# cristianpjensen/thesis-pai-reconstruction

Hardware: AMD Instinct MI355X
Metric: train images/sec (256x256, bs=64) Pix2Pix step (higher is better)
Workload: dtype bf16; 1 GPU; Pix2Pix generator+PatchGAN GAN step, 256x256x1 pairs, 64 images/GPU (BASELINE configs[1]); global_batch=64, per_gpu_batch=64, loss_type=gan, parallelism=dp1, grad_bucket_dtype=f32

## Files before the change

### include/pai_hip.h

```cpp
#ifndef PAI_HIP_H
#define PAI_HIP_H

#include <stdint.h>

#ifdef __cplusplus
extern "C" {
#endif

#define PAI_F32 0
#define PAI_BF16 1
#define PAI_U8 2

#define PAI_ACT_NONE 0
#define PAI_ACT_LRELU 1
#define PAI_ACT_RELU 2
#define PAI_ACT_TANH 3
#define PAI_ACT_SILU 4

const char* pai_last_error(void);
int pai_version(void);
int pai_build_flags(void);
int pai_device_info(int* cu_count, int* lds_bytes, char* arch_name, int arch_name_len);

#define PAI_TUNABLE_UNSET (-2147483647 - 1)
int pai_set_tunable(const char* name, int value);

typedef struct pai_conv_desc {
    int32_t dtype;
    int32_t transposed;
    int32_t N, H, W;
    int32_t C1, C2;
    int32_t Cout;
    int32_t kernel;
    int32_t stride;
    int32_t pad;
    int32_t relu1, relu2;
    int32_t epilogue_act;
    int32_t groups;
    int32_t pack_flags;
    int32_t hints;
} pai_conv_desc;
#define PAI_HINT_SOLO 1

int pai_conv_out_hw(const pai_conv_desc* d, int* OH, int* OW);
int pai_conv_fwd_stats_rows(const pai_conv_desc* d);
int pai_conv_fwd_stats_rows_max(const pai_conv_desc* d);
int pai_bn_stats_buffer_rows(int rows);

int pai_conv_kernel_id(const pai_conv_desc* d, int op);
int pai_conv_kernel_name(const pai_conv_desc* d, int op, char* name, int name_len);

int pai_create(int device_id, void** handle_out);
int pai_bind(void* handle);
int pai_destroy(void* handle);
int pai_handle_set_workspace(void* handle, void* zeroed_device_memory, int64_t bytes);
int pai_handle_set_scratch(void* handle, void* device_memory, int64_t bytes);
int pai_handle_set_wgrad_workspace(void* handle, void* device_memory, int64_t bytes);

int pai_set_workspace(void* zeroed_device_memory, int64_t bytes);
int64_t pai_conv_workspace_bytes(const pai_conv_desc* d, int op);
int pai_set_scratch(void* device_memory, int64_t bytes);
int64_t pai_conv_scratch_bytes(const pai_conv_desc* d, int op);
int pai_set_wgrad_workspace(void* device_memory, int64_t bytes);
int64_t pai_conv_wgrad_workspace_bytes(const pai_conv_desc* d);

int pai_conv_fwd(const pai_conv_desc* d, const void* x1, const void* x2, const void* w_fwd,
                 const float* bias, void* y_raw, void* y_act, float* y_f32, float* stats,
                 void* stream);

int pai_conv_dgrad(const pai_conv_desc* d, const void* dy, const void* w_dgrad, void* dx1,
                   void* dx2, int only_c2, void* stream);

int pai_conv_dgrad_f32add_ok(const pai_conv_desc* d);
int pai_conv_dgrad_f32add(const pai_conv_desc* d, const void* dy, const void* w_dgrad, const float* addend,
                          float* dx2_f32, void* stream);

int pai_conv_dgrad_act(const pai_conv_desc* d, const void* dy, const void* w_dgrad, void* dx1,
                       void* dx2, const void* a1, int act1, void* stream);

typedef struct pai_bwd_epilogue {
    const void* z;
    const void* add;
    const float* scale;
    const float* shift;
    const float* mean;
    const float* rstd;
    float* partials;
    int32_t act1, act2;
} pai_bwd_epilogue;
int pai_conv_dgrad_bn_rows_max(const pai_conv_desc* d);
int pai_conv_dgrad_bn(const pai_conv_desc* d, const void* dy, const void* w_dgrad, void* dx1,
                      void* dx2, const pai_bwd_epilogue* e, int* partial_rows, void* stream);

typedef struct pai_bn_train {
    const float* gamma;
    const float* beta;
    float eps, momentum;
    int32_t n_updates;
    float* running_mean;
    float* running_var;
    int64_t* num_batches_tracked;
    float *mean, *rstd, *scale, *shift;
} pai_bn_train;
int pai_conv_fwd_bn(const pai_conv_desc* d, const void* x1, const void* x2, const void* w_fwd, const float* bias,
                    void* z, void* a, int act, const pai_bn_train* bn, float* stats, void* stream);
int pai_conv_dgrad_bn_apply(const pai_conv_desc* d, const void* dy, const void* w_dgrad, void* du_scratch, void* dx2,
                            const pai_bwd_epilogue* e, const float* gamma, float* sums, float* dgamma, float* dbeta,
                            void* dz, void* stream);
int pai_conv_bn_fused(const pai_conv_desc* d, int op);

int pai_conv_wgrad(const pai_conv_desc* d, const void* x1, const void* x2, const void* dy,
                   float* dw, float* dbias, void* stream);
int pai_conv_wgrad_overwrite(const pai_conv_desc* d, const void* x1, const void* x2, const void* dy,
                             float* dw, float* dbias, void* stream);
int pai_conv_wgrad_overwrite_w(const pai_conv_desc* d, const void* x1, const void* x2, const void* dy,
                               float* dw, float* dbias, void* stream);

int pai_conv_prologue_ok(const pai_conv_desc* d);
int pai_conv_fwd_pro(const pai_conv_desc* d, const void* x1, const void* w_fwd, const float* bias, void* y_raw,
                     float* stats, const float* pre_scale, const float* pre_shift, int pre_act, void* stream);
int pai_conv_wgrad_pro(const pai_conv_desc* d, const void* x1, const void* dy, float* dw, float* dbias, int overwrite,
                       const float* pre_scale, const float* pre_shift, int pre_act, void* stream);

int pai_pack_weights(int dtype, const float* w_master, int Cout, int taps, int Cin,
                     void* w_fwd_or_null, void* w_dgrad_or_null, void* stream);
int pai_pack_weights_multi(int n, const float* const* w_master, const int32_t* cout, const int32_t* taps,
                           const int32_t* cin, void* const* w_fwd, void* const* w_dgrad, void* stream);

int pai_bn_finalize(const float* stats, int rows, int C, int64_t count, const float* gamma,
                    const float* beta, float eps, float momentum, int n_updates,
                    float* running_mean, float* running_var, int64_t* num_batches_tracked,
                    float* mean, float* rstd, float* scale, float* shift, void* stream);
int pai_bn_eval_coeffs(int C, const float* gamma, const float* beta, const float* running_mean,
                       const float* running_var, float eps, float* scale, float* shift,
                       void* stream);
int pai_bn_apply(int dtype, const void* z, int64_t M, int C, const float* scale,
                 const float* shift, int act, void* out, void* stream);
int pai_bn2_add_act(int dtype, const void* za, const float* scale_a, const float* shift_a, const void* zb,
                    const float* scale_b, const float* shift_b, int64_t M, int C, int act_a, int act, void* out,
                    void* stream);
int pai_bn_bwd_partial_rows(int64_t M);
int pai_bn_bwd_reduce(int dtype, const void* g1, int act1, const void* g2, int act2, const void* a,
                      const void* z, int64_t M, int C, const float* mean, const float* rstd,
                      void* du, float* partials, float* sums, float* dgamma, float* dbeta,
                      void* stream);
int pai_bn_bwd_reduce_affine(int dtype, const void* g1, int act1, const void* g2, int act2, const void* z,
                             int64_t M, int C, const float* scale, const float* shift, const float* mean,
                             const float* rstd, void* du, float* partials, float* sums, float* dgamma,
                             float* dbeta, void* stream);
int pai_bn_bwd_finalize(const float* partials, int rows, int C, float* sums, float* dgamma,
                        float* dbeta, void* stream);
int pai_bn_bwd_apply(int dtype, const void* du, const void* z, int64_t M, int C,
                     const float* mean, const float* rstd, const float* gamma,
                     const float* sums, void* dz, void* stream);
int pai_bn_bwd_apply_affine(int dtype, const void* g1, int act1, const void* z, int64_t M, int C, const float* scale,
                            const float* shift, const float* mean, const float* rstd, const float* gamma,
                            const float* sums, void* dz, void* stream);
int pai_act_bwd(int dtype, const void* g1, int act1, const void* g2, int act2, const void* a,
                int64_t numel, void* du, void* stream);

int pai_dropout2d(int dtype, const void* x, const float* mask, int N, int64_t HW, int C, void* out,
                  void* stream);

int pai_maxpool2(int dtype, const void* x, int N, int H, int W, int C, void* out, unsigned char* idx, void* stream);
int pai_maxpool2_bwd(int dtype, const void* dout, const unsigned char* idx, int N, int H, int W, int C, void* dx,
                     void* stream);
int pai_upsample2(int dtype, const void* x, int N, int H, int W, int C, void* out, void* stream);
int pai_upsample2_bwd(int dtype, const void* dout, int N, int H, int W, int C, void* dx, void* stream);
int pai_add_act(int dtype, const void* a, const void* b, int64_t numel, int act, void* out, void* stream);
int pai_bn2_bwd_reduce(int dtype, const void* d, int act_a, const void* za, const void* zb, int64_t M, int C,
                       const float* scale_a, const float* shift_a, const float* mean_a, const float* rstd_a,
                       const float* mean_b, const float* rstd_b, float* part_a, float* part_b, float* sums_a, float* sums_b,
                       void* stream);
int pai_bn2_bwd_apply(int dtype, const void* d, int act_a, const void* za, const void* zb, int64_t M, int C,
                      const float* scale_a, const float* shift_a, const float* mean_a, const float* rstd_a,
                      const float* gamma_a, const float* sums_a, const float* mean_b, const float* rstd_b,
                      const float* gamma_b, const float* sums_b, void* dza, void* dzb, void* stream);
int pai_instnorm_fwd(int dtype, const void* x, int N, int HW, int C, float eps, int act, void* y, float* mean, float* rstd,
                     void* stream);
int pai_instnorm_bwd(int dtype, const void* g, const void* x, int N, int HW, int C, int act, const float* mean,
                     const float* rstd, void* dx, void* stream);

int pai_layernorm_partial_rows(int64_t M);
int pai_layernorm_fwd(int dtype, const void* x, const void* res, int64_t M, int D, const float* gamma,
                      const float* beta, float eps, const float* post, int P, void* sum_out, void* y,
                      float* mean, float* rstd, void* stream);
int pai_layernorm_bwd(int dtype, const void* dy, const void* xs, int64_t M, int D, const float* gamma,
                      const float* mean, const float* rstd, void* dx, float* dgamma_dbeta, float* partials,
                      void* stream);
int pai_gelu(int dtype, const void* z, int64_t numel, void* out, void* stream);
int pai_gelu_bwd(int dtype, const void* dy, const void* z, int64_t numel, void* dz, void* stream);
int pai_mha_fwd(int dtype, const void* qkv, int S, int B, int heads, int hd, const float* mask, void* out,
                float* probs, void* stream);
int pai_mha_bwd(int dtype, const void* dout, const void* qkv, const float* probs, int S, int B, int heads,
                int hd, const float* mask, void* dqkv, float* ds_workspace, void* stream);
int pai_mha_kernel_name(int dtype, int S, int hd, int op, char* name, int name_len);
int pai_subsample2(int dtype, const void* x, int N, int H, int W, int C, void* out, void* stream);
int pai_subsample2_bwd(int dtype, const void* dout, int N, int H, int W, int C, void* dx, void* stream);
int pai_bn_stats_rows(int64_t M);
int pai_bn_stats(int dtype, const void* z, int64_t M, int C, float* stats, void* stream);
int pai_colsum(int dtype, const void* x, int64_t rows, int C, float* out, void* stream);

int pai_gate_partial_rows(int64_t M);
int pai_gate_hidden(int dtype, const void* ig, const void* sg, int64_t M, int K, const float* scale_i,
                    const float* shift_i, const float* scale_s, const float* shift_s, const float* w_a,
                    const float* b_a, void* h, float* logit, float* partials, void* stream);
int pai_gate_apply(int dtype, const void* x, const float* logit, int64_t M, int C, const float* scale_a,
                   const float* shift_a, void* out, float* att, void* stream);
int pai_gate_apply_bwd(int dtype, const void* dout, const void* x, const float* att, const float* logit,
                       int64_t M, int C, const float* mean_a, const float* rstd_a, void* dx_skip, float* dl,
                       float* partials, int relu_out, void* stream);
int pai_gate_hidden_bwd(int dtype, const float* dl, const float* logit, const void* h, const void* ig,
                        const void* sg, int64_t M, int K, const float* mean_a, const float* rstd_a,
                        const float* gamma_a, const float* sums_a, const float* w_a, const float* mean_i,
                        const float* rstd_i, const float* mean_s, const float* rstd_s, void* dsum,
                        float* partials_i, float* partials_s, float* dw_a, float* db_a, void* stream);

int pai_bce_logits(const float* logits, int64_t numel, float target, float loss_scale,
                   double* loss, float grad_scale, float* grad, void* stream);
int pai_l1(const float* pred, const float* target, int64_t numel, float loss_scale, double* loss,
           float grad_scale, float* grad, void* stream);
int pai_mse(const float* pred, const float* target, int64_t numel, float loss_scale, double* loss,
            float grad_scale, float* grad, void* stream);
int pai_head_loss_ok(const pai_conv_desc* d, int has_bias);
int pai_head_loss(const pai_conv_desc* d, const void* a3, const void* w_fwd, const void* w_dgrad, int n_first,
                  float target_first, float target_rest, float loss_scale, double* loss, float grad_scale,
                  float* logits, void* dl, float* dl_f32, void* du, const void* act_src, int act, void* stream);
int pai_scalar_take(double* acc, float* out, void* stream);
int pai_metrics_take(double* sums, int64_t n_images, int64_t numel, float* out3, void* stream);
int pai_tanh_bwd(int dtype, const float* pred, const float* g_a, const float* g_b, int64_t numel,
                 void* dh, void* stream);

int pai_denormalize(const float* x, const float* grad_out_or_null, int64_t numel, float* out,
                    void* stream);

int pai_ssim_sse(const float* pred, const float* target, int NC, int H, int W, int denorm,
                 double* out2, double* per_image, float* full_map, void* stream);
int pai_ssim_psnr_bwd(const float* pred, const float* target, int NC, int H, int W, int denorm,
                      float w_ssim, float w_psnr, const double* sse, float* grad, float* workspace,
                      void* stream);
int64_t pai_ssim_bwd_workspace_floats(int NC, int H, int W);
int pai_eval_planes(const float* pred, const float* target, int NC, int H, int W, int denorm,
                    double* ssim_plane, double* sse_plane, unsigned char* ssim_map_u8,
                    const unsigned char* lut_rgb, unsigned char* hot_u8, void* stream);
int pai_eval_kernel_name(int op, char* name, int name_len);

int pai_cast(int src_dtype, const void* src, int dst_dtype, void* dst, int64_t numel, void* stream);
int pai_reduce_rows(const float* partial, int rows, int C, float* out, int accumulate, void* stream);
int pai_adam(float* param, const float* grad, float* exp_avg, float* exp_avg_sq, int64_t numel,
             float lr, float beta1, float beta2, float eps, int step_count, void* stream);
int pai_adam_pack(float* param, const float* grad, float* exp_avg, float* exp_avg_sq, int64_t numel, int64_t w_off,
                  int Cout, int taps, int Cin, void* w_fwd, void* w_dgrad, float lr, float beta1, float beta2, float eps,
                  int step_count, void* stream);
int pai_adam_dev(float* param, const float* grad, float* exp_avg, float* exp_avg_sq, int64_t numel,
                 float lr, float beta1, float beta2, float eps, int64_t* step_dev, float* coeff2_dev, void* stream);
int pai_adam_multi(int count, void* const* params, const void* const* grads, void* const* exp_avgs,
                   void* const* exp_avg_sqs, const int64_t* numels, float lr, float beta1, float beta2, float eps,
                   int step_count, void* stream);
int pai_adam_multi_dev(int count, void* const* params, const void* const* grads, void* const* exp_avgs,
                       void* const* exp_avg_sqs, const int64_t* numels, float lr, float beta1, float beta2, float eps,
                       int64_t* step_dev, float* coeff2_dev, void* stream);

#define PAI_COMM_ID_BYTES 128
int pai_comm_unique_id(void* id_out_host);
int pai_comm_init(const void* id_host, int rank, int world, void** comm_out);
int pai_allreduce(void* comm, void* ptr, int64_t count, int dtype, void* stream);
int pai_comm_destroy(void* comm);

typedef struct pai_plan_s* pai_plan_t;
int pai_plan_create(pai_plan_t* out);
int pai_plan_destroy(pai_plan_t plan);
int pai_plan_begin(pai_plan_t plan);
int pai_plan_end(pai_plan_t plan);
int pai_plan_run(pai_plan_t plan, int64_t step_delta);
int pai_plan_info(pai_plan_t plan, int* launches, int* waits, int* streams, int64_t* runs);
int pai_stream_wait(void* waiting_stream, void* signalling_stream);
int pai_stream_wait_last(void* waiting_stream, void* signalling_stream);
typedef struct pai_event_s* pai_event_t;
int pai_event_create(pai_event_t* out);
int pai_event_destroy(pai_event_t ev);
int pai_event_record(pai_event_t ev, void* stream);
int pai_event_create_timing(pai_event_t* out);
int pai_event_elapsed_ms(pai_event_t start, pai_event_t stop, float* ms_host);
int pai_profile_arm(pai_event_t start, pai_event_t stop);
int pai_stream_wait_event(void* waiting_stream, pai_event_t ev);
int pai_zero_multi(int count, void* const* ptrs, const int64_t* numels, void* stream);
int pai_cast_multi(int count, int src_dtype, const void* const* srcs, int dst_dtype, void* const* dsts,
                   const int64_t* numels, void* stream);
int pai_lerp_multi(int count, void* const* dsts, const void* const* srcs, const int64_t* numels, float weight, void* stream);

int pai_filter_to_dense(const float* w_oihw, int Cout, int Cin_per_group, int taps, int groups, float* dense, void* stream);
int pai_filter_grad_from_dense(const float* dense_dw, int Cout, int Cin_per_group, int taps, int groups, float* dw_oihw,
                               void* stream);

int pai_swap_mid(int elem_bytes, const void* src, int64_t A, int B, int C, int64_t D, void* dst, void* stream);
int pai_scale(float* ptr, int64_t numel, float factor, void* stream);

int pai_resize_aa_u8(const void* src, int n, int H, int W, int S, const int* wbounds, const float* wweights, int KW,
                     const int* hbounds, const float* hweights, int KH, const int* hbounds_host, void* dst, void* stream);
int pai_batch_gather(int src_dtype, const void* cache_a, const void* cache_b, int64_t M, int64_t per_image,
                     const int64_t* indices, int count, const float* table, float* out_a, float* out_b, void* stream);
int pai_data_kernel_name(int op, int src_dtype, char* name, int name_len);

int pai_sattn_fwd(int dtype, const void* qkv, int N, int T, int heads, int ch, void* out, void* stream);
int pai_sattn_fwd_lse(int dtype, const void* qkv, int N, int T, int heads, int ch, void* out, float* lse, void* stream);
int pai_sattn_bwd(int dtype, const void* dout, const void* qkv, const void* out, const float* lse, int N, int T, int heads,
                  int ch, void* dqkv, float* ws, void* stream);
int pai_sattn_kernel_name(int dtype, int ch, int op, char* name, int name_len);
int pai_affine_act(int dtype, const void* x, int64_t rows_per_sample, int N, int C, const float* A, const float* B,
                   int per_sample, int act, void* out, void* stream);
// ... 22 lines not shown
```

### thesis-pai-reconstruction_amd/csrc/api.hip

```cpp
#include <stdarg.h>

#include "common.h"

static thread_local char g_err[512] = "";

void pai_set_error(const char* fmt, ...) {
    va_list ap;
    va_start(ap, fmt);
    vsnprintf(g_err, sizeof(g_err), fmt, ap);
    va_end(ap);
}

extern "C" const char* pai_last_error(void) { return g_err; }
extern "C" int pai_version(void) { return 140; }

extern "C" int pai_build_flags(void) { return 0; }

extern "C" int pai_device_info(int* cu_count, int* lds_bytes, char* arch_name, int arch_name_len) {
    int dev = 0;
    hipError_t e = hipGetDevice(&dev);
    PAI_CHECK(e == hipSuccess, "hipGetDevice: %s", hipGetErrorString(e));
    hipDeviceProp_t p;
    e = hipGetDeviceProperties(&p, dev);
    PAI_CHECK(e == hipSuccess, "hipGetDeviceProperties: %s", hipGetErrorString(e));
    if (cu_count) *cu_count = p.multiProcessorCount;
    if (lds_bytes) *lds_bytes = (int)p.sharedMemPerBlock;
    if (arch_name && arch_name_len > 0) {
        strncpy(arch_name, p.gcnArchName, arch_name_len - 1);
        arch_name[arch_name_len - 1] = 0;
    }
    return 0;
}

struct Tunable { char name[32]; int value; };
static Tunable g_tunables[32];
static int g_ntunables = 0;

struct TunableEnv { char name[32]; int has, value; };
static TunableEnv g_tunable_env[48];
static int g_ntunable_env = 0;
static bool tunable_env(const char* name, int* value) {
    for (int i = 0; i < g_ntunable_env; ++i)
        if (!strcmp(g_tunable_env[i].name, name)) { *value = g_tunable_env[i].value; return g_tunable_env[i].has != 0; }
    char key[64];
    snprintf(key, sizeof(key), "PAI_TUNE_%s", name);
    const char* e = getenv(key);
    if (g_ntunable_env < 48 && strlen(name) < sizeof(g_tunable_env[0].name)) {
        TunableEnv& t = g_tunable_env[g_ntunable_env];
        strcpy(t.name, name);
        t.has = e != nullptr;
        t.value = e ? atoi(e) : 0;
        ++g_ntunable_env;
    }
    *value = e ? atoi(e) : 0;
    return e != nullptr;
}

int pai_tunable(const char* name, int def) {
    for (int i = 0; i < g_ntunables; ++i)
        if (!strcmp(g_tunables[i].name, name)) return g_tunables[i].value;
    int v;
    return tunable_env(name, &v) ? v : def;
}

extern "C" int pai_set_tunable(const char* name, int value) {
    PAI_CHECK(name && strlen(name) < sizeof(g_tunables[0].name), "pai_set_tunable: bad name");
    for (int i = 0; i < g_ntunables; ++i)
        if (!strcmp(g_tunables[i].name, name)) {
            if (value == PAI_TUNABLE_UNSET) g_tunables[i] = g_tunables[--g_ntunables];
            else g_tunables[i].value = value;
            return 0;
        }
    if (value == PAI_TUNABLE_UNSET) return 0;
    PAI_CHECK(g_ntunables < 32, "pai_set_tunable: table full");
    strcpy(g_tunables[g_ntunables].name, name);
    g_tunables[g_ntunables++].value = value;
    return 0;
}

static void finish_gg(GG* g);

static int check_desc(const pai_conv_desc* d) {
    PAI_CHECK(d != nullptr, "null descriptor");
    PAI_CHECK(d->dtype == PAI_F32 || d->dtype == PAI_BF16, "bad dtype %d", d->dtype);
    if (d->kernel == 1) {
        PAI_CHECK(d->pad == 0 && d->stride == 1 && !d->transposed, "kernel=1 needs pad=0 stride=1 Conv2d");
    } else if (d->kernel == 3) {
        PAI_CHECK(d->pad == 1 && d->stride == 1 && !d->transposed, "kernel=3 needs pad=1 stride=1 Conv2d");
    } else {
        PAI_CHECK(d->kernel == 4 && d->pad == 1, "only kernel=4 pad=1 or kernel=1 pad=0 supported (got k=%d p=%d)",
                  d->kernel, d->pad);
    }
    PAI_CHECK(d->N > 0 && d->H > 0 && d->W > 0 && d->C1 > 0 && d->C2 >= 0 && d->Cout > 0,
              "bad shape N=%d H=%d W=%d C1=%d C2=%d Cout=%d", d->N, d->H, d->W, d->C1, d->C2,
              d->Cout);
    if (d->transposed) {
        PAI_CHECK(d->stride == 2, "ConvTranspose2d needs stride 2");
// ... 467 lines not shown

extern "C" int pai_conv_fwd_pro(const pai_conv_desc* d, const void* x1, const void* w_fwd, const float* bias, void* y_raw,
                                float* stats, const float* pre_scale, const float* pre_shift, int pre_act, void* stream) {
    GG g;
    if (gg_build_fwd(d, &g)) return 1;
    PAI_CHECK(x1 && w_fwd && y_raw && pre_scale && pre_shift, "pai_conv_fwd_pro: null pointer");
    PAI_CHECK(pre_act == PAI_ACT_NONE || pre_act == PAI_ACT_RELU, "pai_conv_fwd_pro: pre_act=%d (none or ReLU)", pre_act);
    PAI_CHECK(d->C2 == 0, "pai_conv_fwd_pro: one source tensor only");
    FwdArgs a;
    memset(&a, 0, sizeof(a));
    a.x1 = x1; a.w = w_fwd; a.bias = bias;
    a.y1 = y_raw;
    a.stats = stats;
    a.pscale = pre_scale; a.pshift = pre_shift; a.pact = pre_act;
    return run_fwd(d->dtype, g, a, (hipStream_t)stream);
}

extern "C" int pai_conv_wgrad_pro(const pai_conv_desc* d, const void* x1, const void* dy, float* dw, float* dbias,
                                  int overwrite, const float* pre_scale, const float* pre_shift, int pre_act, void* stream) {
    PAI_CHECK(pre_scale && pre_shift, "pai_conv_wgrad_pro: null prologue");
    PAI_CHECK(pre_act == PAI_ACT_NONE || pre_act == PAI_ACT_RELU, "pai_conv_wgrad_pro: pre_act=%d (none or ReLU)", pre_act);
    PAI_CHECK(d->C2 == 0, "pai_conv_wgrad_pro: one source tensor only");
    return conv_wgrad_impl(d, x1, nullptr, dy, dw, dbias, overwrite ? 1 : 0, stream, pre_scale, pre_shift, pre_act);
}

extern "C" int pai_conv_dgrad(const pai_conv_desc* d, const void* dy, const void* w_dgrad,
                              void* dx1, void* dx2, int only_c2, void* stream) {
    GG g;
    if (gg_build_dgrad(d, &g)) return 1;
    PAI_CHECK(dy && w_dgrad, "pai_conv_dgrad: null dy / w");
    PAI_CHECK(only_c2 ? (dx2 && d->C2 > 0) : (dx1 != nullptr), "pai_conv_dgrad: missing output");
    PAI_CHECK(d->C2 == 0 || dx2, "pai_conv_dgrad: C2 > 0 but dx2 is null");
    FwdArgs a;
    memset(&a, 0, sizeof(a));
    a.x1 = dy; a.w = w_dgrad;
    a.y1 = dx1; a.y2 = dx2;
    a.skip_d1 = only_c2;
    return run_fwd(d->dtype, g, a, (hipStream_t)stream);
}

extern "C" int pai_conv_dgrad_f32add_ok(const pai_conv_desc* d) {
    GG g;
    if (!d || gg_build_dgrad(d, &g)) return 0;
    return pai_tunable("head_fused", 1) && thin_up_f32add_ok(d->dtype, g) ? 1 : 0;
}

extern "C" int pai_conv_dgrad_f32add(const pai_conv_desc* d, const void* dy, const void* w_dgrad, const float* addend,
                                     float* dx2_f32, void* stream) {
    GG g;
    if (gg_build_dgrad(d, &g)) return 1;
    PAI_CHECK(dy && w_dgrad && addend && dx2_f32, "pai_conv_dgrad_f32add: null pointer");
    PAI_CHECK(thin_up_f32add_ok(d->dtype, g), "pai_conv_dgrad_f32add: not a bf16 (1 | 1)-channel k4 s2 layer on thin_up_k (ask pai_conv_dgrad_f32add_ok)");
    FwdArgs a;
    memset(&a, 0, sizeof(a));
    a.x1 = dy; a.w = w_dgrad;
    a.yf32 = dx2_f32; a.badd = addend;
    a.skip_d1 = 1;
    return launch_thin_dgrad(g, a, (hipStream_t)stream);
}

extern "C" int pai_conv_dgrad_act(const pai_conv_desc* d, const void* dy, const void* w_dgrad,
                                  void* dx1, void* dx2, const void* a1, int act1, void* stream) {
    GG g;
    if (gg_build_dgrad(d, &g)) return 1;
    PAI_CHECK(dy && w_dgrad && dx1 && a1, "pai_conv_dgrad_act: null pointer");
    PAI_CHECK(d->C2 == 0 || dx2, "pai_conv_dgrad_act: C2 > 0 but dx2 is null");
    PAI_CHECK(act1 == PAI_ACT_LRELU || act1 == PAI_ACT_RELU || act1 == PAI_ACT_NONE, "pai_conv_dgrad_act: act1=%d", act1);
    FwdArgs a;
    memset(&a, 0, sizeof(a));
    a.x1 = dy; a.w = w_dgrad;
    a.y1 = dx1; a.y2 = dx2;
    hipStream_t s = (hipStream_t)stream;
    FwdPick p = pick_fwd(d->dtype, g, a);
    const bool fused = p.fused || p.k == FK_HEAD_DGRAD;
    if (fused) {
        a.bz = a1; a.bact1 = act1;
        p = pick_fwd(d->dtype, g, a);
    }
    int rc = run_fwd(p, d->dtype, g, a, s);
    if (rc || fused || act1 == PAI_ACT_NONE) return rc;
    return pai_act_bwd(d->dtype, dx1, act1, nullptr, PAI_ACT_NONE, a1, (int64_t)g.N * g.OH * g.OW * g.D1, dx1, stream);
}

extern "C" int pai_conv_dgrad_bn_rows_max(const pai_conv_desc* d) {
    GG g;
    if (gg_build_dgrad(d, &g)) return -1;
    int fused = cdiv(g.M, 16) * g.nphase;
    if (pw_rows(g) > fused) fused = pw_rows(g);
    if (pwx_rows(g) > fused) fused = pwx_rows(g);
    const int twopass = pai_bn_bwd_partial_rows((int64_t)g.N * g.OH * g.OW);
    return fused > twopass ? fused : twopass;
}

int bn_bwd_reduce_affine(int dtype, void* g1_du, int act1, const void* g2, int act2, const void* z, int64_t M, int C,
                         const float* scale, const float* shift, const float* mean, const float* rstd,
                         float* partials, hipStream_t s);

extern "C" int pai_conv_dgrad_bn(const pai_conv_desc* d, const void* dy, const void* w_dgrad, void* dx1,
                                 void* dx2, const pai_bwd_epilogue* e, int* partial_rows, void* stream) {
    GG g;
    if (gg_build_dgrad(d, &g)) return 1;
    PAI_CHECK(dy && w_dgrad && dx1 && e && e->z, "pai_conv_dgrad_bn: null pointer");
    PAI_CHECK(d->C2 == 0 || dx2, "pai_conv_dgrad_bn: C2 > 0 but dx2 is null");
    PAI_CHECK((e->scale == nullptr) == (e->shift == nullptr), "pai_conv_dgrad_bn: scale and shift go together");
    PAI_CHECK(!e->partials || (e->mean && e->rstd && partial_rows), "pai_conv_dgrad_bn: partials need mean, rstd and partial_rows");
    for (int act : {e->act1, e->act2})
        PAI_CHECK(act == PAI_ACT_LRELU || act == PAI_ACT_RELU || act == PAI_ACT_NONE, "pai_conv_dgrad_bn: act=%d", act);
    FwdArgs a;
    memset(&a, 0, sizeof(a));
    a.x1 = dy; a.w = w_dgrad;
    a.y1 = dx1; a.y2 = dx2;
    hipStream_t s = (hipStream_t)stream;
    const int64_t M = (int64_t)g.N * g.OH * g.OW;
    const FwdPick plain = pick_fwd(d->dtype, g, a);
    if (plain.fused) {
        a.bz = e->z; a.badd = e->add;
        a.bscale = e->scale; a.bshift = e->shift; a.bmean = e->mean; a.brstd = e->rstd;
        a.bact1 = e->act1; a.bact2 = e->act2;
        a.bpart = e->partials;
        const FwdPick p = pick_fwd(d->dtype, g, a);
        PAI_CHECK(p.fused, "pai_conv_dgrad_bn: no kernel with the fused store takes this epilogue");
        if (partial_rows) *partial_rows = e->partials ? p.rows : 0;
        return run_fwd(p, d->dtype, g, a, s);
    }
    if (e->partials) {
        if (const int rows = thin_fwd_bwd_rows(d->dtype, g, a, e->act1, e->add, e->scale)) {
            a.bz = e->z; a.bmean = e->mean; a.brstd = e->rstd; a.bpart = e->partials; a.bact1 = e->act1;
            *partial_rows = rows;
            return run_fwd(d->dtype, g, a, s);
        }
    }
    int rc = run_fwd(plain, d->dtype, g, a, s);
    if (rc) return rc;
    if (e->partials) {
        *partial_rows = pai_bn_bwd_partial_rows(M);
        return bn_bwd_reduce_affine(d->dtype, dx1, e->act1, e->add, e->act2, e->z, M, g.D1, e->scale, e->shift,
                                    e->mean, e->rstd, e->partials, s);
    }
    if (partial_rows) *partial_rows = 0;
    PAI_CHECK(e->scale == nullptr, "pai_conv_dgrad_bn: affine pre-activation without partial sums is only built for the matrix-core kernels");
    return pai_act_bwd(d->dtype, dx1, e->act1, e->add, e->act2, e->z, M * g.D1, dx1, stream);
}

extern "C" int pai_conv_fwd_bn(const pai_conv_desc* d, const void* x1, const void* x2, const void* w_fwd, const float* bias,
                               void* z, void* a_out, int act, const pai_bn_train* bn, float* stats, void* stream) {
    GG g;
    if (gg_build_fwd(d, &g)) return 1;
    PAI_CHECK(x1 && w_fwd && z && a_out && bn && stats, "pai_conv_fwd_bn: null pointer");
    PAI_CHECK(d->C2 == 0 || x2, "pai_conv_fwd_bn: C2 > 0 but x2 is null");
    PAI_CHECK(bn->mean && bn->rstd && bn->scale && bn->shift, "pai_conv_fwd_bn: mean / rstd / scale / shift outputs are required");
    PAI_CHECK(act == PAI_ACT_NONE || act == PAI_ACT_RELU || act == PAI_ACT_LRELU, "pai_conv_fwd_bn: act=%d", act);
    FwdArgs a;
    memset(&a, 0, sizeof(a));
    a.x1 = x1; a.x2 = x2; a.w = w_fwd; a.bias = bias;
    a.y1 = z; a.stats = stats;
    a.eact = PAI_ACT_NONE;
    hipStream_t s = (hipStream_t)stream;
    const int64_t count = (int64_t)g.N * g.OH * g.OW;
    const FwdPick p = pick_fwd(d->dtype, g, a);
    if (int rc = run_fwd(p, d->dtype, g, a, s)) return rc;
    const int rows = p.rows;
    if (bn_fuse_small_ok(rows, count, g.Cout))
        return launch_bn_fin_apply(d->dtype, stats, rows, g.Cout, count, bn->gamma, bn->beta, bn->eps, bn->momentum,
                                   bn->n_updates, bn->running_mean, bn->running_var, bn->num_batches_tracked, bn->mean,
                                   bn->rstd, bn->scale, bn->shift, z, act, a_out, s);
    if (int rc = pai_bn_finalize(stats, rows, g.Cout, count, bn->gamma, bn->beta, bn->eps, bn->momentum, bn->n_updates,
// ... 88 lines not shown
```

### thesis-pai-reconstruction_amd/csrc/gg_mfma.hip

```cpp
#include <type_traits>

#include "gg_tile.h"


bool fwd_mfma_ok(int dtype, const GG& g, const FwdArgs& a) {
    if (dtype != PAI_BF16) return false;
    if (g.C1 % 64 || g.C2 % 64) return false;
    if (g.Cout % 64) return false;
    if (g.D2 > 0 && (g.D1 % 64)) return false;
    if (a.yf32) return false;
    if (a.skip_d1) return false;
    if ((a.y1 || a.y2) && a.yact) return false;
    if (a.yact && a.eact != PAI_ACT_NONE && a.eact != PAI_ACT_LRELU && a.eact != PAI_ACT_RELU) return false;
    return true;
}

struct FwdCfg { int bn, ksplit; };

static FwdCfg fwd_cfg(const GG& g) {
    FwdCfg c;
    c.bn = ((g.Cout % 128) == 0 && (g.D2 == 0 || (g.D1 % 128) == 0)) ? 128 : 64;
    c.ksplit = 1;
    const int ntiles = g.Cout / c.bn;
    const int niter = g.ntaps * g.Cin / MBK;
// ... 199 lines not shown
            relu_cur = relu_next;
        }
    } else {
        for (int it = 0; it < niter; ++it) {
            relu_cur = fire(0);
            if (it + 1 < niter) prepare();
            __syncthreads();
            compute(0, relu_cur);
            __syncthreads();
        }
    }

    if (SPLITK) {
        float* dst = ws + ((size_t)(ks * g.nphase + ph) * g.M + m0) * g.Cout + n0;
#pragma unroll
        for (int mt = 0; mt < MT; ++mt)
#pragma unroll
            for (int r = 0; r < 4; ++r) {
                const int row = wm * WR + mt * 16 + fq * 4 + r;
                if (m0 + row < g.M) {
#pragma unroll
                    for (int nt = 0; nt < NT; ++nt)
                        dst[(size_t)row * g.Cout + wn * (BN / 2) + nt * 16 + fr] = acc[mt][nt][r];
                }
            }
        return;
    }

    constexpr int CROW = BN * 2 + 16;
    constexpr int WM = BM / WR;
    unsigned char* Cs = smem;
    float* sstat = (float*)(smem + BM * CROW);
    const float eslope = act_slope(a.yact ? a.eact : PAI_ACT_NONE);
    float csum[NT], csq[NT];
#pragma unroll
    for (int nt = 0; nt < NT; ++nt) {
        const int col = wn * (BN / 2) + nt * 16 + fr;
        const float b = a.bias ? a.bias[n0 + col] : 0.f;
        float s = 0.f, q = 0.f;
#pragma unroll
        for (int mt = 0; mt < MT; ++mt) {
#pragma unroll
            for (int r = 0; r < 4; ++r) {
                const int row = wm * WR + mt * 16 + fq * 4 + r;
                float v = acc[mt][nt][r] + b;
                if (m0 + row < g.M) { s += v; q += v * v; }
                v = act_fwd(v, eslope);
                *(bf16_t*)(Cs + row * CROW + col * 2) = f2bf(v);
            }
        }
        csum[nt] = s;
        csq[nt] = q;
    }
    if (a.stats) {
#pragma unroll
        for (int nt = 0; nt < NT; ++nt) {
            float s = csum[nt], q = csq[nt];
            s += __shfl_xor(s, 16, 64); s += __shfl_xor(s, 32, 64);
            q += __shfl_xor(q, 16, 64); q += __shfl_xor(q, 32, 64);
            if (fq == 0) {
                const int col = wn * (BN / 2) + nt * 16 + fr;
                sstat[(wm * 2 + 0) * BN + col] = s;
                sstat[(wm * 2 + 1) * BN + col] = q;
            }
        }
    }
    __syncthreads();
    if (a.stats && tid < BN) {
        float* dst = a.stats + ((size_t)(ph * mtiles + bm) * 2) * g.Cout + n0 + tid;
        float s = 0.f, q = 0.f;
#pragma unroll
        for (int i = 0; i < WM; ++i) { s += sstat[(i * 2 + 0) * BN + tid]; q += sstat[(i * 2 + 1) * BN + tid]; }
        dst[0] = s;
        dst[g.Cout] = q;
    }
    bf16_t* dst;
    int dstride, dcol;
    if (a.yact) { dst = (bf16_t*)a.yact; dstride = g.Cout; dcol = n0; }
    else if (n0 < g.D1) { dst = (bf16_t*)a.y1; dstride = g.D1; dcol = n0; }
    else { dst = (bf16_t*)a.y2; dstride = g.D2; dcol = n0 - g.D1; }
    const bool bwd = a.bz && !a.yact && n0 < g.D1;
    const bf16_t* bzp = (const bf16_t*)a.bz;
    const bf16_t* bap = (const bf16_t*)a.badd;
    const bool bsum = bwd && a.bpart;
    constexpr int CPR = BN / 8;
    constexpr int ORP = NTHR / CPR;
    const int oc = tid % CPR, orow0 = tid / CPR;
    BwdParams BP;
    float bs1[8], bs2[8];
#pragma unroll
    for (int k = 0; k < 8; ++k) bs1[k] = bs2[k] = 0.f;
    constexpr int NP = BM / ORP, NB = NP < 4 ? NP : 4;
    if (bwd) bwd_load_params(a, dcol + oc * 8, BP);
#pragma unroll
    for (int p0 = 0; p0 < NP; p0 += NB) {
        size_t offs[NB];
        uint4 zq[NB], aq[NB];
#pragma unroll
        for (int p = 0; p < NB; ++p) {
            const int m = m0 + orow0 + (p0 + p) * ORP;
            int n, gy, gx;
            decode_row(g, m < g.M ? m : 0, n, gy, gx);
            const size_t pix = (size_t)(n * g.OH + gy * g.OS + g.poy[ph]) * g.OW + gx * g.OS + g.pox[ph];
            offs[p] = pix * dstride + dcol + oc * 8;
            if (bwd) {
                zq[p] = *(const uint4*)(bzp + offs[p]);
                aq[p] = bap ? *(const uint4*)(bap + offs[p]) : make_uint4(0, 0, 0, 0);
            }
        }
#pragma unroll
        for (int p = 0; p < NB; ++p) {
            const int row = orow0 + (p0 + p) * ORP;
            if (m0 + row < g.M) {
                uint4 o = *(const uint4*)(Cs + row * CROW + oc * 16);
                if (bwd)
                    o = bwd_chunk(o, zq[p], aq[p], bap != nullptr, a.bscale != nullptr, bsum, a.bact1, a.bact2, BP, bs1, bs2);
                *(uint4*)(dst + offs[p]) = o;
            }
        }
    }
    if (bsum)
        bwd_write_partials<BN, CPR, NTHR / 64>(sstat, bs1, bs2, tid,
                                               a.bpart + ((size_t)(ph * mtiles + bm) * 2) * g.D1 + n0, g.D1,
                                               a.bmean + n0, a.brstd + n0);
}

constexpr int FIN_COLS = 128;
__global__ __launch_bounds__(256) void splitk_finish_k(GG g, FwdArgs a, const float* ws, int mtiles, int ksplit) {
    __shared__ float red[2][FIN_ROWS][FIN_COLS + 8];
    const int tid = threadIdx.x;
    const int bm = blockIdx.x, ph = blockIdx.y, cb = blockIdx.z;
    const int row = tid >> 4, cgl = tid & 15;
    const int m = bm * FIN_ROWS + row;
    const int c0 = cb * FIN_COLS + cgl * 8;
    const bool valid = m < g.M && c0 < g.Cout;
    const float eslope = act_slope(a.yact ? a.eact : PAI_ACT_NONE);
    float v[8], bs1[8], bs2[8];
#pragma unroll
    for (int k = 0; k < 8; ++k) v[k] = bs1[k] = bs2[k] = 0.f;
    if (valid) {
        const size_t slab = (size_t)g.nphase * g.M * g.Cout;
        const float* src = ws + ((size_t)ph * g.M + m) * g.Cout + c0;
#pragma unroll 4
        for (int s = 0; s < ksplit; ++s) {
            const float4 v0 = *(const float4*)(src + s * slab), v1 = *(const float4*)(src + s * slab + 4);
            v[0] += v0.x; v[1] += v0.y; v[2] += v0.z; v[3] += v0.w;
            v[4] += v1.x; v[5] += v1.y; v[6] += v1.z; v[7] += v1.w;
        }
        if (a.bias) {
#pragma unroll
            for (int k = 0; k < 8; ++k) v[k] += a.bias[c0 + k];
        }
    }
    if (a.stats) {
#pragma unroll
        for (int k = 0; k < 8; ++k) {
            red[0][row][cgl * 8 + k] = v[k];
            red[1][row][cgl * 8 + k] = v[k] * v[k];
        }
    }
    if (valid) {
        unsigned packed[4];
#pragma unroll
        for (int k = 0; k < 8; ++k) v[k] = act_fwd(v[k], eslope);
#pragma unroll
        for (int k = 0; k < 4; ++k) packed[k] = pk2bf(v[2 * k], v[2 * k + 1]);
        int n, gy, gx;
        decode_row(g, m, n, gy, gx);
        const size_t pix = (size_t)(n * g.OH + gy * g.OS + g.poy[ph]) * g.OW + gx * g.OS + g.pox[ph];
        bf16_t* dst;
        if (a.yact) dst = (bf16_t*)a.yact + pix * g.Cout + c0;
        else if (c0 < g.D1) dst = (bf16_t*)a.y1 + pix * g.D1 + c0;
        else dst = (bf16_t*)a.y2 + pix * g.D2 + (c0 - g.D1);
        uint4 o = make_uint4(packed[0], packed[1], packed[2], packed[3]);
        if (a.bz && !a.yact && c0 < g.D1) {
            BwdParams BP;
            bwd_load_params(a, c0, BP);
            const size_t off = pix * g.D1 + c0;
            const bf16_t* bap = (const bf16_t*)a.badd;
            o = bwd_chunk(o, *(const uint4*)((const bf16_t*)a.bz + off),
                          bap ? *(const uint4*)(bap + off) : make_uint4(0, 0, 0, 0), bap != nullptr,
                          a.bscale != nullptr, a.bpart != nullptr, a.bact1, a.bact2, BP, bs1, bs2);
        }
        *(uint4*)dst = o;
    }
    if (a.stats) {
        __syncthreads();
        const int c = cb * FIN_COLS + tid;
        if (tid < FIN_COLS && c < g.Cout) {
            float t1 = 0.f, t2 = 0.f;
#pragma unroll
            for (int r = 0; r < FIN_ROWS; ++r) { t1 += red[0][r][tid]; t2 += red[1][r][tid]; }
            float* dst = a.stats + ((size_t)(ph * mtiles + bm) * 2) * g.Cout + c;
            dst[0] = t1;
            dst[g.Cout] = t2;
        }
    } else if (a.bpart && a.bz) {
#pragma unroll
        for (int k = 0; k < 8; ++k) {
            red[0][row][cgl * 8 + k] = bs1[k];
            red[1][row][cgl * 8 + k] = bs2[k];
        }
        __syncthreads();
        const int c = cb * FIN_COLS + tid;
        if (tid < FIN_COLS && c < g.D1) {
            float t1 = 0.f, t2 = 0.f;
#pragma unroll
            for (int r = 0; r < FIN_ROWS; ++r) { t1 += red[0][r][tid]; t2 += red[1][r][tid]; }
            float* dst = a.bpart + ((size_t)(ph * mtiles + bm) * 2) * g.D1 + c;
            dst[0] = t1;
            dst[g.D1] = a.brstd[c] * (t2 - a.bmean[c] * t1);
        }
    }
}



static int patch_rows(const GG& g, const FwdCfg& c, PatchGeo* pg) {
    const bool no_256 = !pai_tunable("fwd_patch256", 1);
    if (!pai_tunable("fwd_patch", 1) || c.ksplit > 1) return 0;
    if ((int64_t)g.N * g.H * g.W * (g.C1 > g.C2 ? g.C1 : g.C2) * 2 >= (1ll << 31) || (int64_t)g.Cout * g.wtaps * g.Cin * 2 >= (1ll << 31))
        return 0;
    if (!no_256 && c.bn == 128 && (int64_t)(g.M / 256) * (g.Cout / 128) * g.nphase >= 512 && patch_geo(g, 16, pg)) return 256;
    if (!no_256 && c.bn == 64 && g.Cin >= 256 && pai_tunable("fwd_w1", 1) &&
        (int64_t)(g.M / 256) * (g.Cout / 64) * g.nphase >= pai_tunable("fwd_w1_min", 768) && patch_geo(g, 16, pg))
        return 256;
    return patch_geo(g, 8, pg) ? 128 : 0;
}

#ifndef PATCH_ABL
#define PATCH_ABL 0
#endif
#ifndef EPI_ABL
#define EPI_ABL 0
#endif
#ifndef PATCH_COLSWZ_ALL
#define PATCH_COLSWZ_ALL 0
#endif
#ifndef PATCH_SETPRIO
#define PATCH_SETPRIO 1
#endif
template <int BM, int BN, bool DBB, int WN = 2, int WPX = 64, bool COLSWZ = true>
__device__ __forceinline__ void gg_fwd_patch_body(const GG& g, const FwdArgs& a, const PatchGeo& pg, int mtiles, int ntiles) {
    static_assert(WN == 2 || BN == 64, "one wave column: 64 output channels");
    constexpr int abl = PATCH_ABL;
    typedef PatchDims<BM, WN, WPX> PD;
    constexpr int NTHR = PD::NTHR, MT = WPX / 16, NT = BN / (16 * WN);
    constexpr int BNW = BN / WN;
    constexpr int RPP = PD::RPP, PJ = PD::PJ, PATCH_PIX = PD::PIX, PATCH_BYTES = PD::BYTES;
    constexpr int BJ = BN / RPP;
    extern __shared__ __attribute__((aligned(16))) unsigned char smem[];
    unsigned char* Bs = smem + PATCH_BYTES;

    const int tid = threadIdx.x, lane = tid & 63;
    const int wid = __builtin_amdgcn_readfirstlane(tid >> 6);
    const int wm = WN == 2 ? wid >> 1 : wid, wn = WN == 2 ? wid & 1 : 0;
    int bid = xcd_remap(blockIdx.x, gridDim.x);
    const int bn = bid % ntiles;
    bid /= ntiles;
    const int ph = bid % g.nphase;
    const int bm = bid / g.nphase;
    const int n0 = bn * BN;
    const int tpi = pg.TY * pg.TX;
    const int img = bm / tpi, trem = bm - img * tpi;
    const int gy0 = (trem / pg.TX) * PD::TH, gx0 = (trem % pg.TX) * 16;

    constexpr unsigned OOB = 0x80000000u;
    const __amdgpu_buffer_rsrc_t wrs = __builtin_amdgcn_make_buffer_rsrc(
        const_cast<void*>(a.w), 0, (unsigned)(g.Cout * g.wtaps * g.Cin) * 2u, 0x00020000);
    const unsigned xpix = (unsigned)(g.N * g.H * g.W);
    const __amdgpu_buffer_rsrc_t x1rs = __builtin_amdgcn_make_buffer_rsrc(
        const_cast<void*>(a.x1), 0, xpix * (unsigned)g.C1 * 2u, 0x00020000);
    const __amdgpu_buffer_rsrc_t x2rs = __builtin_amdgcn_make_buffer_rsrc(
        const_cast<void*>(a.x2 ? a.x2 : a.x1), 0, a.x2 ? xpix * (unsigned)g.C2 * 2u : 0u, 0x00020000);
    unsigned wby16 = 0, wbx16 = 0;
#pragma unroll
    for (int q = 0; q < 4; ++q) {
        wby16 |= (unsigned)((pg.by[ph][q] + 8) & 15) << (4 * q);
        wbx16 |= (unsigned)((pg.bx[ph][q] + 8) & 15) << (4 * q);
    }
    wby16 = __builtin_amdgcn_readfirstlane(wby16);
    wbx16 = __builtin_amdgcn_readfirstlane(wbx16);
    const unsigned wtlo = __builtin_amdgcn_readfirstlane(pg.wt_lo[ph]);
    const unsigned wthi = __builtin_amdgcn_readfirstlane(pg.wt_hi[ph]);
    const unsigned toff2 = __builtin_amdgcn_readfirstlane(pg.toff2[ph]);
    const unsigned relu_bits = __builtin_amdgcn_readfirstlane((g.relu1 ? 1u : 0u) | (g.relu2 ? 2u : 0u));

    const int sc = lane & 7, sr = wid * 8 + (lane >> 3);
    unsigned pfill[PJ];
#pragma unroll
    for (int j = 0; j < PJ; ++j) {
        const int p = j * RPP + sr;
        const int py = p / PATCH_W, px = p - py * PATCH_W;
        const int y = (gy0 + py) * g.S, x = (gx0 + px) * g.S;
// ... 162 lines not shown
                if (DBB) {
                    if (k < 3) fire_b(gi, k + 1, buf ^ 1);
                    else if (more) fire_b(gi + 1, 0, buf ^ 1);
                }
                const unsigned bb = b_base + (DBB ? buf * (BN * 128) : 0);
    #pragma unroll
                for (int kk = 0; kk < 2; ++kk) {
                    const unsigned ca = (unsigned)((kk * 4 + fq) << 4);
                    const unsigned cb = (unsigned)(((kk * 4 + fq) ^ fswz) << 4);
                    bf8_t af[MT], bfr[NT];
                    if (!(abl & 8)) {
    #pragma unroll
                        for (int mt = 0; mt < MT; ++mt) af[mt] = *(const bf8_t*)(smem + (abase[mt] ^ ca));
    #pragma unroll
                        for (int nt = 0; nt < NT; ++nt) bfr[nt] = *(const bf8_t*)(smem + bb + nt * 16 * 128 + cb);
                    } else {
    #pragma unroll
                        for (int mt = 0; mt < MT; ++mt) af[mt] = __builtin_bit_cast(bf8_t, make_uint4(ca, cb, mt, kk));
    #pragma unroll
                        for (int nt = 0; nt < NT; ++nt) bfr[nt] = __builtin_bit_cast(bf8_t, make_uint4(cb, ca, nt, kk));
                    }
                    if (relu) {
    #pragma unroll
                        for (int mt = 0; mt < MT; ++mt) af[mt] = relu_frag(af[mt]);
                    }
                    if (PATCH_SETPRIO) __builtin_amdgcn_s_setprio(1);
                    if (!(abl & 4)) {
    #pragma unroll
                        for (int mt = 0; mt < MT; ++mt)
    #pragma unroll
                            for (int nt = 0; nt < NT; ++nt)
                                acc[mt][nt] = __builtin_amdgcn_mfma_f32_16x16x32_bf16(bfr[nt], af[mt], acc[mt][nt], 0, 0, 0);
                    } else {
                        acc[0][0][0] += (float)af[0][0] + (float)bfr[0][0];
                    }
                    if (PATCH_SETPRIO) __builtin_amdgcn_s_setprio(0);
                }
                if (DBB) {
                    buf ^= 1;
                    if (k == 3 && more) {
                        asm volatile("s_waitcnt lgkmcnt(0)" ::: "memory");
                        __builtin_amdgcn_s_barrier();
                        fire_patch(gi + 1);
                    }
                } else {
                    asm volatile("s_waitcnt lgkmcnt(0)" ::: "memory");
                    __builtin_amdgcn_s_barrier();
                    if (k < 3) fire_b(gi, k + 1, 0);
                    else if (more) { fire_patch(gi + 1); fire_b(gi + 1, 0, 0); }
                }
            }
        }
    }
    asm volatile("s_waitcnt lgkmcnt(0)" ::: "memory");
    __builtin_amdgcn_s_barrier();
    if (abl & 16) {
        float t = 0.f;
#pragma unroll
        for (int i = 0; i < MT; ++i)
#pragma unroll
            for (int j = 0; j < NT; ++j) {
                t += acc[i][j][0] + acc[i][j][1] + acc[i][j][2] + acc[i][j][3];
            }
        if (t == 123.456f) *(float*)a.y1 = t;
        return;
    }

    constexpr int CROW = BN * 2 + 16;
    constexpr int WM = BM / WPX;
    unsigned char* Cs = smem;
    float* sstat = (float*)(smem + BM * CROW);
    const int eact = a.yact ? a.eact : PAI_ACT_NONE;
    const float eslope = act_slope(eact);
    constexpr int CL = 4 * NT;
    const int col0 = wn * BNW + CL * fq;
    bf16_t* dst;
    int dstride, dcol;
    if (a.yact) { dst = (bf16_t*)a.yact; dstride = g.Cout; dcol = n0; }
    else if (n0 < g.D1) { dst = (bf16_t*)a.y1; dstride = g.D1; dcol = n0; }
    else { dst = (bf16_t*)a.y2; dstride = g.D2; dcol = n0 - g.D1; }
    const bool bwd = a.bz && !a.yact && n0 < g.D1;
    const bf16_t* bzp = (const bf16_t*)a.bz;
    const bf16_t* bap = (const bf16_t*)a.badd;
    const bool bsum = bwd && a.bpart;
    constexpr int CPR = BN / 8;
    constexpr int ORP = NTHR / CPR;
    static_assert(ORP % 16 == 0, "a pass covers whole 16-pixel tile rows");
    const int oc = tid % CPR, orow0 = tid / CPR;
    constexpr int NP = BM / ORP, NB = NP < 4 ? NP : 4, NBATCH = NP / NB;
    const size_t tile0 = ((size_t)(img * g.OH + gy0 * g.OS + g.poy[ph]) * g.OW + gx0 * g.OS + g.pox[ph]) * dstride + dcol;
    const unsigned toff = (unsigned)((((orow0 >> 4) * g.OS * g.OW + (orow0 & 15) * g.OS) * dstride + oc * 8) * 2);
    const unsigned pstep = (unsigned)((ORP / 16) * g.OS * g.OW * dstride * 2);
    const char* zt = (const char*)(bzp + tile0);
    const char* at = (const char*)(bap + tile0);
    char* dt = (char*)(dst + tile0);
    const float sl1 = act_slope(a.bact1), sl2 = act_slope(a.bact2);
    uint4 zq[NB], aq[NB];
    if (bwd && !(EPI_ABL & 1)) {
#pragma unroll
        for (int p = 0; p < NB; ++p) zq[p] = *(const uint4*)(zt + (toff + (unsigned)p * pstep));
    }
    const bool has_bias = a.bias != nullptr, has_stats = a.stats != nullptr;
    auto stage = [&](auto full_tag) {
        constexpr bool FULL = decltype(full_tag)::value;
        float bias_v[FULL ? CL : 1], csum[FULL ? CL : 1], csq[FULL ? CL : 1];
        if (FULL) {
#pragma unroll
            for (int c = 0; c < CL; ++c) { bias_v[c] = has_bias ? a.bias[n0 + col0 + c] : 0.f; csum[c] = csq[c] = 0.f; }
        }
#pragma unroll
        for (int mt = 0; mt < MT; ++mt) {
            const int row = wm * WPX + mt * 16 + fr;
#pragma unroll
            for (int h = 0; h < CL / 8; ++h) {
                float v[8];
#pragma unroll
                for (int c = 0; c < 8; ++c) {
                    v[c] = acc[mt][(8 * h + c) >> 2][c & 3];
                    if (FULL) {
                        v[c] += bias_v[8 * h + c];
                        csum[8 * h + c] += v[c];
                        csq[8 * h + c] = fmaf(v[c], v[c], csq[8 * h + c]);
                    }
                }
                if (eact != PAI_ACT_NONE) {
#pragma unroll
                    for (int c = 0; c < 8; ++c) v[c] = act_fwd(v[c], eslope);
                }
                *(uint4*)(Cs + row * CROW + (col0 + 8 * h) * 2) =
                    make_uint4(pk2bf(v[0], v[1]), pk2bf(v[2], v[3]), pk2bf(v[4], v[5]), pk2bf(v[6], v[7]));
            }
        }
        if (FULL && has_stats) {
#pragma unroll
            for (int c = 0; c < CL; ++c) {
                float s = csum[c], q = csq[c];
                s += __builtin_bit_cast(float, __builtin_amdgcn_update_dpp(0, __builtin_bit_cast(int, s), 0xB1, 0xF, 0xF, false));
                q += __builtin_bit_cast(float, __builtin_amdgcn_update_dpp(0, __builtin_bit_cast(int, q), 0xB1, 0xF, 0xF, false));
                s += __builtin_bit_cast(float, __builtin_amdgcn_update_dpp(0, __builtin_bit_cast(int, s), 0x4E, 0xF, 0xF, false));
                q += __builtin_bit_cast(float, __builtin_amdgcn_update_dpp(0, __builtin_bit_cast(int, q), 0x4E, 0xF, 0xF, false));
                s += __builtin_bit_cast(float, __builtin_amdgcn_update_dpp(0, __builtin_bit_cast(int, s), 0x141, 0xF, 0xF, false));
                q += __builtin_bit_cast(float, __builtin_amdgcn_update_dpp(0, __builtin_bit_cast(int, q), 0x141, 0xF, 0xF, false));
                s += __builtin_bit_cast(float, __builtin_amdgcn_update_dpp(0, __builtin_bit_cast(int, s), 0x140, 0xF, 0xF, false));
                q += __builtin_bit_cast(float, __builtin_amdgcn_update_dpp(0, __builtin_bit_cast(int, q), 0x140, 0xF, 0xF, false));
                if (fr == 0) {
                    sstat[(wm * 2 + 0) * BN + col0 + c] = s;
                    sstat[(wm * 2 + 1) * BN + col0 + c] = q;
                }
            }
        }
    };
    if (has_bias || has_stats) stage(std::true_type{});
    else stage(std::false_type{});
    if (bwd && bap) {
#pragma unroll
        for (int p = 0; p < NB; ++p) aq[p] = *(const uint4*)(at + (toff + (unsigned)p * pstep));
    }
    BwdParams BP;
    float bs1[8], bs2[8];
#pragma unroll
    for (int k = 0; k < 8; ++k) bs1[k] = bs2[k] = 0.f;
    if (bwd) bwd_load_params(a, dcol + oc * 8, BP);
    __syncthreads();
    if (has_stats && tid < BN) {
        float* dst = a.stats + ((size_t)(ph * mtiles + bm) * 2) * g.Cout + n0 + tid;
        float s = 0.f, q = 0.f;
#pragma unroll
        for (int i = 0; i < WM; ++i) { s += sstat[(i * 2 + 0) * BN + tid]; q += sstat[(i * 2 + 1) * BN + tid]; }
        dst[0] = s;
        dst[g.Cout] = q;
    }
    auto store_tile = [&](auto bwd_tag, auto add_tag, auto sum_tag) {
        constexpr bool BWD = decltype(bwd_tag)::value, ADD = decltype(add_tag)::value, SUM = decltype(sum_tag)::value;
        auto request = [&](int pass, int slot) {
            const unsigned off = toff + (unsigned)pass * pstep;
            if (BWD && !(EPI_ABL & 1)) zq[slot] = *(const uint4*)(zt + off);
            if (BWD && ADD) aq[slot] = *(const uint4*)(at + off);
        };
#pragma unroll
        for (int b = 0; b < NBATCH; ++b) {
#pragma unroll
            for (int p = 0; p < NB; ++p) {
                const int pass = b * NB + p;
                uint4 o = *(const uint4*)(Cs + (orow0 + pass * ORP) * CROW + oc * 16);
                if (EPI_ABL & 1) zq[p] = o;
                if (BWD && !(EPI_ABL & 2)) o = bwd_chunk_t<ADD, SUM>(o, zq[p], aq[p], sl1, sl2, BP, bs1, bs2);
                if (BWD && (EPI_ABL & 2)) { o.x ^= zq[p].x; if (ADD) o.y ^= aq[p].y; }
                if (b + 1 < NBATCH) request(pass + NB, p);
                if (!(EPI_ABL & 4) || o.x == 0x12345u) *(uint4*)(dt + (toff + (unsigned)pass * pstep)) = o;
                __builtin_amdgcn_sched_barrier(0);
            }
        }
    };
    typedef std::true_type T_;
    typedef std::false_type F_;
    if (!bwd) store_tile(F_{}, F_{}, F_{});
    else if (bap) { if (bsum) store_tile(T_{}, T_{}, T_{}); else store_tile(T_{}, T_{}, F_{}); }
    else { if (bsum) store_tile(T_{}, F_{}, T_{}); else store_tile(T_{}, F_{}, F_{}); }
    if (bsum)
        bwd_write_partials<BN, CPR, NTHR / 64>(sstat, bs1, bs2, tid,
                                               a.bpart + ((size_t)(ph * mtiles + bm) * 2) * g.D1 + n0, g.D1,
                                               a.bmean + n0, a.brstd + n0);
}

template <int BM, int BN, bool DBB>
__global__ __launch_bounds__(BM * 2, (BM == 128 && DBB) ? (BN == 64 ? 4 : 3) : (BN == 64 ? 5 : 4)) void gg_fwd_patch_k(GG g, FwdArgs a, PatchGeo pg, int mtiles, int ntiles) {
    gg_fwd_patch_body<BM, BN, DBB, 2, 64, PATCH_COLSWZ_ALL || !(BN == 128 && (BM == 256 || !DBB))>(g, a, pg, mtiles, ntiles);
}
template <int BM, int BN, bool DBB>
__global__ __launch_bounds__(BM, 3) void gg_fwd_patch1_k(GG g, FwdArgs a, PatchGeo pg, int mtiles, int ntiles) {
    gg_fwd_patch_body<BM, BN, DBB, 1>(g, a, pg, mtiles, ntiles);
}
static size_t fwd_lds_bytes(int bm, int bn, bool db) {
    const size_t main_loop = (size_t)(db ? 2 : 1) * (bm * 128 + bn * 128);
    const size_t epilogue = bm * (bn * 2 + 16) + (bm / 64 * 2) * 2 * bn * sizeof(float);
    return main_loop > epilogue ? main_loop : epilogue;
}

#define FWD_MFMA_VARIANTS(X)                                         \
    X(FWD_SPLITK128_DB, TILE, gg_fwd_mfma_k, 128, 128, true, true, 64)   \
    X(FWD_SPLITK128, TILE, gg_fwd_mfma_k, 128, 128, true, false, 64)     \
    X(FWD_SPLITK64, TILE, gg_fwd_mfma_k, 128, 64, true, false, 64)       \
    X(FWD_PATCH1_256, PATCH, gg_fwd_patch1_k, 256, 64, false)            \
    X(FWD_PATCH256_DBB, PATCH, gg_fwd_patch_k, 256, 128, true)           \
    X(FWD_PATCH128_DBB, PATCH, gg_fwd_patch_k, 128, 128, true)           \
    X(FWD_PATCH128N, PATCH, gg_fwd_patch_k, 128, 64, false)              \
    X(FWD_TILE128, TILE, gg_fwd_mfma_k, 128, 128, false, false, 64)      \
    X(FWD_TILE64, TILE, gg_fwd_mfma_k, 128, 64, false, false, 64)
#define X(id, form, k, ...) id,
enum FwdMfmaVariant { FWD_MFMA_VARIANTS(X) };
#undef X
#define X(id, form, k, ...) #k "<" #__VA_ARGS__ ">",
static const char* const fwd_mfma_names[] = {FWD_MFMA_VARIANTS(X)};
#undef X

MfmaPlan fwd_mfma_plan(const GG& g) {
    MfmaPlan p = {};
    FwdCfg c = fwd_cfg(g);
    p.workspace_bytes = c.ksplit > 1 ? (int64_t)c.ksplit * g.nphase * g.M * g.Cout * 4 : 0;
    if (c.ksplit > 1 && (pai_ctx()->workspace == nullptr || pai_ctx()->workspace_bytes < p.workspace_bytes)) c.ksplit = 1;
    p.ksplit = c.ksplit;
    p.bm = 128;
    p.bn = c.bn;
    p.mtiles = cdiv(g.M, p.bm);
    p.ntiles = g.Cout / c.bn;
    const int prow = patch_rows(g, c, &p.pg);
    p.rows = c.ksplit > 1 ? cdiv(g.M, FIN_ROWS) : (prow == 256 ? g.M / 256 : p.mtiles);
    int waves = 0;
    bool db = false;
    size_t patch_bytes = 0;
    if (c.ksplit > 1) {
        db = c.bn == 128 && pai_tunable("fwd_splitk_db", 1);
        p.variant = c.bn == 64 ? FWD_SPLITK64 : (db ? FWD_SPLITK128_DB : FWD_SPLITK128);
    } else if (prow == 256 && c.bn == 64) {
        waves = 4; patch_bytes = PatchDims<256, 1>::BYTES;
        p.variant = FWD_PATCH1_256;
    } else if (prow == 256) {
        db = true; waves = 8; patch_bytes = PatchDims<256>::BYTES;
        p.variant = FWD_PATCH256_DBB;
    } else if (prow == 128) {
        db = c.bn == 128; waves = 4; patch_bytes = PatchDims<128>::BYTES;
        p.variant = db ? FWD_PATCH128_DBB : FWD_PATCH128N;
    } else p.variant = c.bn == 128 ? FWD_TILE128 : FWD_TILE64;
    p.db = db;
    p.name = fwd_mfma_names[p.variant];
    if (waves) {
        p.bm = prow;
        p.mtiles = g.M / prow;
        p.block = waves * 64;
        const size_t lds = patch_bytes + (size_t)c.bn * 128 * (db ? 2 : 1);
        const size_t epi = prow * ((size_t)c.bn * 2 + 16) + waves * 2 * c.bn * sizeof(float);
        p.lds = lds > epi ? lds : epi;
    } else {
        p.block = p.bm / 64 * 128;
        p.lds = fwd_lds_bytes(p.bm, c.bn, db);
    }
    p.grid = p.mtiles * p.ntiles * g.nphase * c.ksplit;
    return p;
}

static int fwd_lds_opt_in();
int launch_fwd_mfma(const GG& g, const FwdArgs& a, const MfmaPlan& p, hipStream_t s) {
    float* ws = pai_ctx()->workspace;
    if (p.lds > 64 * 1024 && fwd_lds_opt_in()) return 1;
#define FWD_LAUNCH_TILE(k, ...) PAI_LAUNCH((k<__VA_ARGS__>), p.grid, p.block, p.lds, s, g, a, p.mtiles, p.ntiles, p.ksplit, ws)
// ... 712 lines not shown
```

### thesis-pai-reconstruction_amd/csrc/gg_tile.h

```cpp
#pragma once
#include <stdlib.h>

#include "common.h"

typedef __attribute__((ext_vector_type(8))) __bf16 bf8_t;
typedef __attribute__((ext_vector_type(4))) __bf16 bf4_t;
typedef __attribute__((ext_vector_type(4))) float f4_t;
typedef __attribute__((ext_vector_type(2))) short s2_t;
typedef __attribute__((ext_vector_type(4))) unsigned u4_t;

constexpr int MBK = 64;

static __device__ uint4 g_zero_line[16];

#define GLDS16(gptr, lptr)                                                                      \
    __builtin_amdgcn_global_load_lds((const __attribute__((address_space(1))) void*)(gptr),    \
                                     (__attribute__((address_space(3))) void*)(lptr), 16, 0, 0)

typedef __attribute__((ext_vector_type(8))) short s8_t;

#ifndef RELU_ABL
#define RELU_ABL 0
#endif
__device__ __forceinline__ bf8_t relu_frag(bf8_t f) {
    if (RELU_ABL) return f;
    s8_t x = __builtin_bit_cast(s8_t, f);
    const s8_t z = {0, 0, 0, 0, 0, 0, 0, 0};
    x = __builtin_elementwise_max(x, z);
    return __builtin_bit_cast(bf8_t, x);
}

__device__ __forceinline__ void decode_row(const GG& g, int m, int& n, int& gy, int& gx) {
    if (g.lw >= 0) {
        gx = m & (g.OWg - 1);
        gy = (m >> g.lw) & (g.OHg - 1);
        n = m >> (g.lw + g.lh);
    } else {
        gx = m % g.OWg;
        int r = m / g.OWg;
        gy = r % g.OHg;
        n = r / g.OHg;
    }
}

__device__ __forceinline__ int xcd_remap(int bid, int nwg) {
    const int q = nwg >> 3, r = nwg & 7, x = bid & 7;
    return (x < r ? x * (q + 1) : r * (q + 1) + (x - r) * q) + (bid >> 3);
}

struct BwdParams { float sc[8], sh[8]; };
static __device__ const float g_unit_affine[16] = {1.f, 1.f, 1.f, 1.f, 1.f, 1.f, 1.f, 1.f, 0.f, 0.f, 0.f, 0.f, 0.f, 0.f, 0.f, 0.f};
__device__ __forceinline__ void bwd_load_params(const FwdArgs& a, int c, BwdParams& P) {
    const float* sp = a.bscale ? a.bscale + c : g_unit_affine;
    const float* hp = a.bscale ? a.bshift + c : g_unit_affine + 8;
    const float4 s0 = *(const float4*)sp, s1 = *(const float4*)(sp + 4);
    const float4 h0 = *(const float4*)hp, h1 = *(const float4*)(hp + 4);
    P.sc[0] = s0.x; P.sc[1] = s0.y; P.sc[2] = s0.z; P.sc[3] = s0.w; P.sc[4] = s1.x; P.sc[5] = s1.y; P.sc[6] = s1.z; P.sc[7] = s1.w;
    P.sh[0] = h0.x; P.sh[1] = h0.y; P.sh[2] = h0.z; P.sh[3] = h0.w; P.sh[4] = h1.x; P.sh[5] = h1.y; P.sh[6] = h1.z; P.sh[7] = h1.w;
}
__device__ __forceinline__ float bwd_sel(float g, bool pos, float slope) {
    const float sg = slope == 0.f ? 0.f : fmaf(g, slope, 0.f);
    return pos ? g : sg;
}
template <bool HAS_ADD, bool SUMS>
__device__ __forceinline__ uint4 bwd_chunk_t(uint4 gq, uint4 zq, uint4 aq, float sl1, float sl2, const BwdParams& P,
                                             float* s1, float* s2) {
    const unsigned gw[4] = {gq.x, gq.y, gq.z, gq.w}, zw[4] = {zq.x, zq.y, zq.z, zq.w}, aw[4] = {aq.x, aq.y, aq.z, aq.w};
    unsigned o[4];
#pragma unroll
    for (int k = 0; k < 4; ++k) {
        const float g0 = __uint_as_float(gw[k] << 16), g1 = __uint_as_float(gw[k] & 0xffff0000u);
        const float z0 = __uint_as_float(zw[k] << 16), z1 = __uint_as_float(zw[k] & 0xffff0000u);
        const bool q0 = fmaf(z0, P.sc[2 * k], P.sh[2 * k]) > 0.f;
        const bool q1 = fmaf(z1, P.sc[2 * k + 1], P.sh[2 * k + 1]) > 0.f;
        float d0 = bwd_sel(g0, q0, sl1), d1 = bwd_sel(g1, q1, sl1);
        if (HAS_ADD) {
            d0 += bwd_sel(__uint_as_float(aw[k] << 16), q0, sl2);
            d1 += bwd_sel(__uint_as_float(aw[k] & 0xffff0000u), q1, sl2);
        }
        o[k] = pk2bf(d0, d1);
        if (SUMS) {
            const float r0 = __uint_as_float(o[k] << 16), r1 = __uint_as_float(o[k] & 0xffff0000u);
            s1[2 * k] += r0;
            s1[2 * k + 1] += r1;
            s2[2 * k] = fmaf(r0, z0, s2[2 * k]);
            s2[2 * k + 1] = fmaf(r1, z1, s2[2 * k + 1]);
        }
    }
    return make_uint4(o[0], o[1], o[2], o[3]);
}
__device__ __forceinline__ uint4 bwd_chunk(uint4 gq, uint4 zq, uint4 aq, bool has_add, bool , bool sums,
                                           int act1, int act2, const BwdParams& P, float* s1, float* s2) {
    const float sl1 = act_slope(act1), sl2 = act_slope(act2);
    if (has_add) return sums ? bwd_chunk_t<true, true>(gq, zq, aq, sl1, sl2, P, s1, s2)
                             : bwd_chunk_t<true, false>(gq, zq, aq, sl1, sl2, P, s1, s2);
    return sums ? bwd_chunk_t<false, true>(gq, zq, aq, sl1, sl2, P, s1, s2)
                : bwd_chunk_t<false, false>(gq, zq, aq, sl1, sl2, P, s1, s2);
}
template <int BN, int CPR, int NW>
__device__ __forceinline__ void bwd_write_partials(float* sred, const float* s1, const float* s2, int tid,
                                                   float* row_dst, int D1, const float* mean, const float* rstd) {
    const int lane = tid & 63, wid = tid >> 6;
#pragma unroll
    for (int k = 0; k < 8; ++k) {
        float a = s1[k], b = s2[k];
#pragma unroll
        for (int o = CPR; o < 64; o <<= 1) { a += __shfl_xor(a, o, 64); b += __shfl_xor(b, o, 64); }
        if (lane < CPR) {
            sred[(wid * 2 + 0) * BN + lane * 8 + k] = a;
            sred[(wid * 2 + 1) * BN + lane * 8 + k] = b;
        }
    }
    __syncthreads();
    if (tid < BN) {
        float a = 0.f, b = 0.f;
#pragma unroll
        for (int w = 0; w < NW; ++w) { a += sred[(w * 2 + 0) * BN + tid]; b += sred[(w * 2 + 1) * BN + tid]; }
        row_dst[tid] = a;
        row_dst[D1 + tid] = rstd[tid] * (b - mean[tid] * a);
    }
}

constexpr int PATCH_W = 17;
template <int BM, int WN = 2, int WPX = 64> struct PatchDims {
    static constexpr int TH = BM / 16;
    static constexpr int PIX = (TH + 1) * PATCH_W;
    static constexpr int NTHR = BM / WPX * 64 * WN;
    static constexpr int RPP = NTHR / 8;
    static constexpr int PJ = (PIX + RPP - 1) / RPP;
    static constexpr int BYTES = PJ * RPP * 128;
};

static inline void patch_geo_pack(PatchGeo* pg) {
    for (int ph = 0; ph < 4; ++ph) {
        pg->wt_lo[ph] = pg->wt_hi[ph] = pg->toff2[ph] = 0;
        for (int q = 0; q < 4; ++q)
            for (int k = 0; k < 4; ++k) {
                const unsigned slot = (pg->wt4[ph][q] >> (8 * k)) & 15u, to = (pg->toff4[ph][q] >> (8 * k)) & 0xffu;
                if (q < 2) pg->wt_lo[ph] |= slot << (16 * q + 4 * k); else pg->wt_hi[ph] |= slot << (16 * (q - 2) + 4 * k);
                pg->toff2[ph] |= ((to / PATCH_W) * 2u + (to % PATCH_W)) << (8 * q + 2 * k);
            }
    }
}
static inline bool patch_geo_raw(const GG& g, int th, PatchGeo* pg, int tw);
static inline bool patch_geo(const GG& g, int th, PatchGeo* pg, int tw = 16) {
    if (!patch_geo_raw(g, th, pg, tw)) return false;
    patch_geo_pack(pg);
    return true;
}
static inline bool patch_geo_raw(const GG& g, int th, PatchGeo* pg, int tw) {
    if ((g.OWg % tw) || (g.OHg % th)) return false;
    memset(pg, 0, sizeof(*pg));
    pg->TY = g.OHg / th;
    pg->TX = g.OWg / tw;
    if (g.S == 1 && g.ntaps == 4) {
        pg->groups = 1;
        for (int ph = 0; ph < g.nphase; ++ph) {
            int by = 127, bx = 127;
            for (int t = 0; t < 4; ++t) { by = g.dy[ph][t] < by ? g.dy[ph][t] : by; bx = g.dx[ph][t] < bx ? g.dx[ph][t] : bx; }
            unsigned seen = 0;
            for (int t = 0; t < 4; ++t) {
                const int ty = g.dy[ph][t] - by, tx = g.dx[ph][t] - bx;
                if (ty > 1 || tx > 1) return false;
                const int k = ty * 2 + tx;
                if (seen & (1u << k)) return false;
                seen |= 1u << k;
                pg->toff4[ph][0] |= (unsigned)(ty * PATCH_W + tx) << (8 * k);
                pg->wt4[ph][0] |= (unsigned)g.wt[ph][t] << (8 * k);
            }
            if (seen != 15u) return false;
            pg->by[ph][0] = (signed char)by;
            pg->bx[ph][0] = (signed char)bx;
        }
        return true;
    }
    if (g.S == 2 && g.ntaps == 16 && g.nphase == 1) {
        pg->groups = 4;
        int ymin = 127, xmin = 127;
        for (int t = 0; t < 16; ++t) { ymin = g.dy[0][t] < ymin ? g.dy[0][t] : ymin; xmin = g.dx[0][t] < xmin ? g.dx[0][t] : xmin; }
        for (int q = 0; q < 4; ++q) {
            const int by = ymin + (q >> 1), bx = xmin + (q & 1);
            int n = 0;
            unsigned seen = 0;
            for (int t = 0; t < 16; ++t) {
                const int ry = g.dy[0][t] - by, rx = g.dx[0][t] - bx;
                if (ry < 0 || rx < 0 || (ry & 1) || (rx & 1)) continue;
                const int ty = ry / 2, tx = rx / 2;
                if (ty > 1 || tx > 1 || n == 4) return false;
                const int k = ty * 2 + tx;
                if (seen & (1u << k)) return false;
                seen |= 1u << k;
                pg->toff4[0][q] |= (unsigned)(ty * PATCH_W + tx) << (8 * k);
                pg->wt4[0][q] |= (unsigned)g.wt[0][t] << (8 * k);
                ++n;
            }
            if (n != 4 || seen != 15u) return false;
            pg->by[0][q] = (signed char)by;
            pg->bx[0][q] = (signed char)bx;
        }
        return true;
    }
    return false;
// ... 35 lines not shown
```

### thesis-pai-reconstruction_amd/csrc/head.hip

```cpp
#include "common.h"

typedef __attribute__((ext_vector_type(8))) __bf16 bf8_t;
typedef __attribute__((ext_vector_type(4))) float f4_t;

constexpr int HL_THREADS = 512, HL_WAVES = HL_THREADS / 64;
constexpr int HL_LD = 17;
constexpr int64_t HL_LDS_MAX = 96 * 1024;

struct HeadLoss {
    const bf16_t* a3;
    const bf16_t* wf;
    const bf16_t* wd;
    float* logits;
    bf16_t* dl;
    float* dl32;
    bf16_t* du;
    const bf16_t* act_src;
    double* loss;
    int N, H, W, C, OH, OW;
    int n_first;
    float t_first, t_rest;
    double ls_first, ls_rest;
    float gs_first, gs_rest;
    int act;
    int rg;
    int xcd;
};

static int64_t head_loss_lds_bytes(int H, int W, int C, bool with_du) {
    const int64_t ys = (((int64_t)H * W * HL_LD * 4) + 15) & ~(int64_t)15;
    const int64_t dls = (((int64_t)(H - 1) * (W - 1) * 4) + 15) & ~(int64_t)15;
    return ys + dls + (with_du ? (int64_t)16 * C * 2 : 0);
}

template <int KS>
__global__ __launch_bounds__(HL_THREADS) void head_loss_k(HeadLoss p) {
    extern __shared__ __attribute__((aligned(16))) unsigned char hl_sm[];
    __shared__ double wsum[HL_WAVES];
    const int P = p.H * p.W, Q = p.OH * p.OW;
    float* Ys = (float*)hl_sm;
    float* dls = (float*)(hl_sm + ((((size_t)P * HL_LD * 4) + 15) & ~(size_t)15));
    bf16_t* wt = (bf16_t*)((unsigned char*)dls + ((((size_t)Q * 4) + 15) & ~(size_t)15));
    const int tid = threadIdx.x, lane = tid & 63, wid = tid >> 6;
    const int fr = lane & 15, fq = lane >> 4;
    int n, rg;
    if (p.xcd) {
        n = (blockIdx.x & 7) + 8 * (blockIdx.x / (8 * p.rg));
        rg = (blockIdx.x >> 3) % p.rg;
    } else {
        n = blockIdx.x / p.rg;
        rg = blockIdx.x - n * p.rg;
    }
    const bool first = n < p.n_first;
    const float tconst = first ? p.t_first : p.t_rest;
    const float gscale = first ? p.gs_first : p.gs_rest;

    if (p.du) {
        for (int i = tid; i < p.C * 16; i += HL_THREADS) {
            const int c = i >> 4, t = i & 15;
            wt[t * p.C + c] = p.wd[i];
        }
    }
    bf8_t af[KS];
#pragma unroll
    for (int s = 0; s < KS; ++s) af[s] = *(const bf8_t*)(p.wf + (size_t)fr * p.C + 32 * s + 8 * fq);
    const bf16_t* x = p.a3 + (size_t)n * P * p.C;
    for (int p0 = wid * 16; p0 < P; p0 += HL_WAVES * 16) {
        const int m = min(p0 + fr, P - 1);
        bf8_t bfr[KS];
#pragma unroll
        for (int s = 0; s < KS; ++s) bfr[s] = *(const bf8_t*)(x + (size_t)m * p.C + 32 * s + 8 * fq);
        f4_t acc = (f4_t){0.f, 0.f, 0.f, 0.f};
#pragma unroll
        for (int s = 0; s < KS; ++s) acc = __builtin_amdgcn_mfma_f32_16x16x32_bf16(af[s], bfr[s], acc, 0, 0, 0);
        if (p0 + fr < P) {
#pragma unroll
            for (int r = 0; r < 4; ++r) Ys[(p0 + fr) * HL_LD + 4 * fq + r] = acc[r];
        }
    }
    __syncthreads();
    double lsum = 0.0;
    for (int i = tid; i < Q; i += HL_THREADS) {
        const int oy = i / p.OW, ox = i - oy * p.OW;
        float v = 0.f;
#pragma unroll
        for (int k = 0; k < 16; ++k) {
            const int iy = oy + (k >> 2) - 1, ix = ox + (k & 3) - 1;
            if ((unsigned)iy < (unsigned)p.H && (unsigned)ix < (unsigned)p.W) v += Ys[(iy * p.W + ix) * HL_LD + k];
        }
        const float xv = v;
        const float l = fmaxf(xv, 0.f) - xv * tconst + log1pf(expf(-fabsf(xv)));
        const float g = 1.f / (1.f + expf(-xv)) - tconst;
        const float gs = g * gscale;
        const bf16_t gb = f2bf(gs);
        dls[i] = bf2f(gb);
        lsum += (double)l;
        if (rg == 0) {
            const size_t o = (size_t)n * Q + i;
            p.logits[o] = xv;
            if (p.dl) p.dl[o] = gb;
            if (p.dl32) p.dl32[o] = gs;
        }
    }
    if (rg == 0) {
        double v = lsum * (first ? p.ls_first : p.ls_rest);
#pragma unroll
        for (int o = 32; o > 0; o >>= 1) v += __shfl_xor(v, o, 64);
        if (lane == 0) wsum[wid] = v;
    }
    __syncthreads();
    if (rg == 0 && tid == 0) {
        double v = wsum[0];
#pragma unroll
        for (int w = 1; w < HL_WAVES; ++w) v += wsum[w];
        if (fabs(v) < 256.0) v = rint(v * 0x1p36) * 0x1p-36;
        atomicAdd(p.loss, v);
    }
    if (!p.du) return;
    const int r0 = (p.H * rg) / p.rg, r1 = (p.H * (rg + 1)) / p.rg;
    const int groups = p.C / 8;
    const int items = (r1 - r0) * p.W * groups;
    for (int item = tid; item < items; item += HL_THREADS) {
        const int pix = item / groups, cg = item - pix * groups;
        const int ry = pix / p.W, ox = pix - ry * p.W, oy = r0 + ry;
        float acc[8];
#pragma unroll
        for (int j = 0; j < 8; ++j) acc[j] = 0.f;
#pragma unroll
        for (int t = 0; t < 16; ++t) {
            const int sy = oy + 1 - (t >> 2), sx = ox + 1 - (t & 3);
            if ((unsigned)sy >= (unsigned)p.OH || (unsigned)sx >= (unsigned)p.OW) continue;
            const float v = dls[sy * p.OW + sx];
            float wv[8];
            V8<bf16_t>::ld(wt + t * p.C + cg * 8, wv);
#pragma unroll
            for (int j = 0; j < 8; ++j) acc[j] = fmaf(v, wv[j], acc[j]);
        }
        const size_t o = ((size_t)n * P + (size_t)oy * p.W + ox) * p.C + cg * 8;
        float zv[8];
        V8<bf16_t>::ld(p.act_src + o, zv);
#pragma unroll
        for (int j = 0; j < 8; ++j) {
            const float gq = bf2f(f2bf(acc[j]));
            acc[j] = p.act == PAI_ACT_NONE ? gq : gq * act_grad(zv[j], p.act);
        }
        V8<bf16_t>::st(p.du + o, acc);
    }
}

static bool head_loss_shape_ok(const pai_conv_desc* d, int has_bias) {
    if (!d || has_bias || d->dtype != PAI_BF16 || d->transposed || d->kernel != 4 || d->stride != 1 || d->pad != 1) return false;
    if (d->Cout != 1 || d->C2 != 0 || d->relu1 || d->epilogue_act != PAI_ACT_NONE || d->groups > 1) return false;
    if (d->N <= 0 || d->H < 2 || d->W < 2 || (d->C1 % 32) != 0) return false;
    const int ks = d->C1 / 32;
    if (!(ks == 1 || ks == 2 || ks == 4 || ks == 8 || ks == 16)) return false;
    return head_loss_lds_bytes(d->H, d->W, d->C1, true) <= HL_LDS_MAX;
}

extern "C" int pai_head_loss_ok(const pai_conv_desc* d, int has_bias) {
    return pai_tunable("head_fused", 1) && head_loss_shape_ok(d, has_bias) ? 1 : 0;
}

extern "C" int pai_head_loss(const pai_conv_desc* d, const void* a3, const void* w_fwd, const void* w_dgrad, int n_first,
                             float target_first, float target_rest, float loss_scale, double* loss, float grad_scale,
                             float* logits, void* dl, float* dl_f32, void* du, const void* act_src, int act, void* stream) {
    PAI_CHECK(head_loss_shape_ok(d, 0), "pai_head_loss: not a bias-free bf16 k4 s1 p1 C -> 1 head within the LDS bound (ask pai_head_loss_ok)");
    PAI_CHECK(a3 && w_fwd && loss && logits, "pai_head_loss: null pointer");
    PAI_CHECK(!du || (w_dgrad && act_src), "pai_head_loss: du needs w_dgrad and act_src");
    PAI_CHECK(act == PAI_ACT_LRELU || act == PAI_ACT_RELU || act == PAI_ACT_NONE, "pai_head_loss: act=%d", act);
    HeadLoss p;
    memset(&p, 0, sizeof(p));
    p.a3 = (const bf16_t*)a3; p.wf = (const bf16_t*)w_fwd; p.wd = (const bf16_t*)w_dgrad;
    p.logits = logits; p.dl = (bf16_t*)dl; p.dl32 = dl_f32; p.du = (bf16_t*)du; p.act_src = (const bf16_t*)act_src;
    p.loss = loss;
    p.N = d->N; p.H = d->H; p.W = d->W; p.C = d->C1; p.OH = d->H - 1; p.OW = d->W - 1;
    p.n_first = n_first < 0 ? 0 : (n_first > d->N ? d->N : n_first);
    p.t_first = target_first; p.t_rest = target_rest;
    const int64_t per = (int64_t)p.OH * p.OW, nf = per * p.n_first, nr = per * (p.N - p.n_first);
    if (nf > 0) { p.ls_first = (double)loss_scale / (double)nf; p.gs_first = (float)((double)grad_scale / (double)nf); }
    if (nr > 0) { p.ls_rest = (double)loss_scale / (double)nr; p.gs_rest = (float)((double)grad_scale / (double)nr); }
    p.act = act;
    int rg = du ? pai_tunable("head_loss_rg", 4) : 1;
    if (rg < 1) rg = 1;
    if (rg > p.H) rg = p.H;
    p.rg = rg;
    p.xcd = (p.N % 8) == 0 ? 1 : 0;
    const size_t lds = (size_t)head_loss_lds_bytes(p.H, p.W, p.C, du != nullptr);
    const dim3 grid((unsigned)(p.N * rg));
    hipStream_t s = (hipStream_t)stream;
#define HL_CASE(KK)                                                                                                     \
    case KK: {                                                                                                          \
        static PerDeviceOnce attr;                                                                                      \
        if (attr.first()) {                                                                                             \
            const hipError_t e = hipFuncSetAttribute(reinterpret_cast<const void*>(&head_loss_k<KK>),                   \
                                                     hipFuncAttributeMaxDynamicSharedMemorySize, (int)HL_LDS_MAX);      \
            PAI_CHECK(e == hipSuccess, "pai_head_loss: hipFuncSetAttribute(max dynamic LDS): %s", hipGetErrorString(e)); \
        }                                                                                                               \
        PAI_LAUNCH(head_loss_k<KK>, grid, dim3(HL_THREADS), lds, s, p);                                                 \
        break;                                                                                                          \
    }
    switch (p.C / 32) {
        HL_CASE(1) HL_CASE(2) HL_CASE(4) HL_CASE(8) HL_CASE(16)
        default: PAI_CHECK(false, "pai_head_loss: unsupported C %d", p.C);
    }
#undef HL_CASE
    PAI_LAUNCH_CHECK();
    return 0;
}
```

### thesis-pai-reconstruction_amd/csrc/misc.hip

```cpp
#include "common.h"

template <typename S, typename D>
__global__ __launch_bounds__(256) void cast_k(const S* src, D* dst, int64_t numel) {
    for (int64_t i = (int64_t)blockIdx.x * 256 + threadIdx.x; i < numel; i += (int64_t)gridDim.x * 256)
        Conv<D>::st(dst + i, Conv<S>::ld(src + i));
}

extern "C" int pai_cast(int src_dtype, const void* src, int dst_dtype, void* dst, int64_t numel,
                        void* stream) {
    PAI_CHECK(src && dst, "pai_cast: null pointer");
    int64_t blocks = (numel + 1023) / 1024;
    if (blocks > 4096) blocks = 4096;
    if (blocks < 1) blocks = 1;
    hipStream_t s = (hipStream_t)stream;
    dim3 g((int)blocks), b(256);
    if (src_dtype == PAI_F32 && dst_dtype == PAI_BF16)
        PAI_LAUNCH((cast_k<float, bf16_t>), g, b, 0, s, (const float*)src, (bf16_t*)dst, numel);
    else if (src_dtype == PAI_BF16 && dst_dtype == PAI_F32)
        PAI_LAUNCH((cast_k<bf16_t, float>), g, b, 0, s, (const bf16_t*)src, (float*)dst, numel);
    else if (src_dtype == PAI_F32 && dst_dtype == PAI_F32)
        PAI_LAUNCH((cast_k<float, float>), g, b, 0, s, (const float*)src, (float*)dst, numel);
    else if (src_dtype == PAI_BF16 && dst_dtype == PAI_BF16)
        PAI_LAUNCH((cast_k<bf16_t, bf16_t>), g, b, 0, s, (const bf16_t*)src, (bf16_t*)dst, numel);
    else
// ... 171 lines not shown
    if (dtype == PAI_BF16 && (Cin % 64) == 0 && (Cout % 64) == 0 && Cout / 64 <= 65535 && taps <= 65535) {
        PAI_LAUNCH(pack64_k, dim3(Cin / 64, Cout / 64, taps), dim3(256), 0, (hipStream_t)stream, w_master, Cout,
                           taps, Cin, (bf16_t*)w_fwd, (bf16_t*)w_dgrad);
        PAI_LAUNCH_CHECK();
        return 0;
    }
    dim3 grid(cdiv(Cin, 32), cdiv(Cout, 32), taps);
    if (dtype == PAI_F32)
        PAI_LAUNCH(pack_k<float>, grid, dim3(256), 0, (hipStream_t)stream, w_master, Cout, taps, Cin,
                           (float*)w_fwd, (float*)w_dgrad);
    else
        PAI_LAUNCH(pack_k<bf16_t>, grid, dim3(256), 0, (hipStream_t)stream, w_master, Cout, taps, Cin,
                           (bf16_t*)w_fwd, (bf16_t*)w_dgrad);
    PAI_LAUNCH_CHECK();
    return 0;
}

__global__ void reduce_rows_k(const float* partial, int rows, int C, float* out, int accumulate) {
    const int c = blockIdx.x * blockDim.x + threadIdx.x;
    if (c >= C) return;
    double s = 0.0;
    for (int r = 0; r < rows; ++r) s += (double)partial[(size_t)r * C + c];
    out[c] = accumulate ? out[c] + (float)s : (float)s;
}

extern "C" int pai_reduce_rows(const float* partial, int rows, int C, float* out, int accumulate,
                               void* stream) {
    PAI_CHECK(partial && out, "pai_reduce_rows: null pointer");
    PAI_LAUNCH(reduce_rows_k, dim3(cdiv(C, 64)), dim3(64), 0, (hipStream_t)stream, partial, rows, C,
                       out, accumulate);
    PAI_LAUNCH_CHECK();
    return 0;
}

template <typename T>
__global__ __launch_bounds__(256) void colsum_k(const T* x, int64_t rows, int C, int64_t rows_per_block,
                                                float* out) {
    __shared__ float red[256];
    const int tid = threadIdx.x;
    const int64_t r0 = (int64_t)blockIdx.x * rows_per_block, r1 = min(rows, r0 + rows_per_block);
    for (int c0 = blockIdx.y * 256; c0 < C; c0 += gridDim.y * 256) {
        const int width = min(C - c0, 256);
        int lanes = 1;
        while (lanes * 2 * width <= 256) lanes *= 2;
        const int c = tid % width, rl = tid / width;
        float s = 0.f;
        if (rl < lanes)
            for (int64_t r = r0 + rl; r < r1; r += lanes) s += Conv<T>::ld(x + r * C + c0 + c);
        red[tid] = (rl < lanes) ? s : 0.f;
        __syncthreads();
        if (tid < width) {
            float t = 0.f;
            for (int l = 0; l < lanes; ++l) t += red[tid + l * width];
            atomicAdd(out + c0 + tid, t);
        }
        __syncthreads();
    }
}

int launch_colsum(int dtype, const void* x, int64_t rows, int C, float* out, hipStream_t s) {
    int64_t blocks = (rows + 255) / 256;
    if (blocks > 512) blocks = 512;
    if (blocks < 1) blocks = 1;
    const int64_t rpb = (rows + blocks - 1) / blocks;
    blocks = (rows + rpb - 1) / rpb;
    int chunks = cdiv(C, 256);
    if (chunks > 64) chunks = 64;
    if (blocks * chunks > 4096) chunks = (int)(4096 / blocks) > 0 ? (int)(4096 / blocks) : 1;
    const dim3 grid((int)blocks, chunks);
    if (dtype == PAI_F32)
        PAI_LAUNCH(colsum_k<float>, grid, dim3(256), 0, s, (const float*)x, rows, C, rpb, out);
    else
        PAI_LAUNCH(colsum_k<bf16_t>, grid, dim3(256), 0, s, (const bf16_t*)x, rows, C, rpb, out);
    PAI_LAUNCH_CHECK();
    return 0;
}

extern "C" int pai_colsum(int dtype, const void* x, int64_t rows, int C, float* out, void* stream) {
    PAI_CHECK(dtype == PAI_F32 || dtype == PAI_BF16, "pai_colsum: bad dtype %d", dtype);
    PAI_CHECK(x && out && rows > 0 && C > 0, "pai_colsum: bad arguments");
    return launch_colsum(dtype, x, rows, C, out, (hipStream_t)stream);
}

__device__ __forceinline__ void adam1(float& p, float& m, float& v, float g, float lr_over_bc1, float beta1, float beta2,
                                      float omb1, float omb2, float eps, float inv_sqrt_bc2) {
#pragma clang fp contract(off)
    const float mi = __builtin_fmaf(beta1, m, omb1 * g);
    const float vi = __builtin_fmaf(beta2, v, omb2 * g * g);
    m = mi;
    v = vi;
    p = p - lr_over_bc1 * mi / __builtin_fmaf(sqrtf(vi), inv_sqrt_bc2, eps);
}

__global__ __launch_bounds__(256) void adam_k(float* p, const float* g, float* m, float* v, int64_t numel,
                                              float lr_over_bc1, float beta1, float beta2, float omb1, float omb2,
                                              float eps, float inv_sqrt_bc2) {
    for (int64_t i = (int64_t)blockIdx.x * 256 + threadIdx.x; i < numel; i += (int64_t)gridDim.x * 256) {
        adam1(p[i], m[i], v[i], g[i], lr_over_bc1, beta1, beta2, omb1, omb2, eps, inv_sqrt_bc2);
    }
}

extern "C" int pai_adam(float* param, const float* grad, float* exp_avg, float* exp_avg_sq, int64_t numel,
                        float lr, float beta1, float beta2, float eps, int step_count, void* stream) {
    PAI_CHECK(param && grad && exp_avg && exp_avg_sq && step_count >= 1, "pai_adam: bad arguments");
    float lr_over_bc1, inv_sqrt_bc2;
    pai::adam_coeffs(lr, beta1, beta2, step_count, &lr_over_bc1, &inv_sqrt_bc2);
    int64_t blocks = (numel + 1023) / 1024;
    if (blocks > 8192) blocks = 8192;
    if (blocks < 1) blocks = 1;
    pai::plan_mark_adam(5, 11, lr, beta1, beta2, step_count);
    PAI_LAUNCH(adam_k, dim3((int)blocks), dim3(256), 0, (hipStream_t)stream, param, grad, exp_avg,
                       exp_avg_sq, numel, lr_over_bc1, beta1, beta2, (float)(1.0 - (double)beta1),
                       (float)(1.0 - (double)beta2), eps, inv_sqrt_bc2);
    PAI_LAUNCH_CHECK();
    return 0;
}

__global__ __launch_bounds__(256) void adam_pack64_k(float* p, const float* g, float* m, float* v, int64_t numel,
                                                     int64_t w_off, int Cout, int taps, int Cin, bf16_t* wf, bf16_t* wd,
                                                     int ntiles, float lr_over_bc1, float beta1, float beta2, float omb1,
                                                     float omb2, float eps, float inv_sqrt_bc2) {
    __shared__ float tile[64][65];
    const int tid = threadIdx.x;
    if ((int)blockIdx.x >= ntiles) {
        const int64_t wn = (int64_t)Cout * taps * Cin;
        const int64_t rest = numel - wn;
        for (int64_t k = (int64_t)(blockIdx.x - ntiles) * 256 + tid; k < rest; k += (int64_t)(gridDim.x - ntiles) * 256) {
            const int64_t i = k < w_off ? k : k + wn;
            adam1(p[i], m[i], v[i], g[i], lr_over_bc1, beta1, beta2, omb1, omb2, eps, inv_sqrt_bc2);
        }
        return;
    }
    const int nci = Cin / 64, nco = Cout / 64;
    const int lb = blockIdx.x;
    const int ci0 = (lb % nci) * 64, co0 = ((lb / nci) % nco) * 64, t = lb / (nci * nco);
    const int q = tid & 15, r0 = tid >> 4;
#pragma unroll
    for (int j = 0; j < 4; ++j) {
        const int r = r0 + 16 * j;
        const int64_t i = w_off + ((int64_t)(co0 + r) * taps + t) * Cin + ci0 + 4 * q;
        const float4 g4 = *(const float4*)(g + i);
        float4 m4 = *(const float4*)(m + i), v4 = *(const float4*)(v + i), p4 = *(const float4*)(p + i);
        float* pe = &p4.x; float* me = &m4.x; float* ve = &v4.x; const float* ge = &g4.x;
#pragma unroll
        for (int e = 0; e < 4; ++e) {
            adam1(pe[e], me[e], ve[e], ge[e], lr_over_bc1, beta1, beta2, omb1, omb2, eps, inv_sqrt_bc2);
            tile[r][4 * q + e] = pe[e];
        }
        *(float4*)(m + i) = m4;
        *(float4*)(v + i) = v4;
        *(float4*)(p + i) = p4;
    }
    __syncthreads();
    const int c = tid & 7, s0 = tid >> 3;
#pragma unroll
    for (int j = 0; j < 2; ++j) {
        const int r = s0 + 32 * j;
        if (wf) {
            unsigned u[4];
#pragma unroll
            for (int e = 0; e < 4; ++e) u[e] = pk2bf(tile[r][8 * c + 2 * e], tile[r][8 * c + 2 * e + 1]);
            *(uint4*)(wf + ((size_t)(co0 + r) * taps + t) * Cin + ci0 + 8 * c) = make_uint4(u[0], u[1], u[2], u[3]);
        }
        if (wd) {
            unsigned u[4];
#pragma unroll
// ... 433 lines not shown
```

### thesis-pai-reconstruction_amd/engine.py

```python
from __future__ import annotations

import os
from typing import Callable, List, Optional

import torch
import torch.nn as nn

from . import ops
from .ops import ACT_LRELU, ACT_NONE, ACT_RELU, ACT_TANH

BN_EPS_DEFAULT = 1e-5


def _fwd_pack_strides(mod) -> tuple:
    if isinstance(mod, nn.ConvTranspose2d):
        cin, cout, kh, kw = mod.weight.shape
        return (1, kh * kw * cin, kw * cin, cin)
    cout, cin, kh, kw = mod.weight.shape
    return (kh * kw * cin, 1, kw * cin, cin)


def _strides_match(t: torch.Tensor, want: tuple) -> bool:
    return all(s == w or n == 1 for s, w, n in zip(t.stride(), want, t.shape))

# ... 738 lines not shown
        P["desc"].append(ops.make_desc(dtype, 0, N, H, W, c, c, self.chans[0], 2, 0, 0, ACT_LRELU))
        for k in range(1, 4):
            P["desc"].append(ops.make_desc(dtype, 0, N, H >> k, W >> k, self.chans[k - 1], 0, self.chans[k], 2, 0, 0,
                                           ACT_LRELU))
        P["desc"].append(ops.make_desc(dtype, 0, N, H >> 4, W >> 4, self.chans[3], 0, 1, 1, 0, 0, ACT_NONE))
        P["oh"], P["ow"] = (H >> 4) - 1, (W >> 4) - 1
        ops.ensure_workspace(max(ops.conv_workspace_bytes(d, op) for d in P["desc"] for op in (0, 1)), device)
        ops.ensure_scratch(ops.scratch_bytes_for(P["desc"]), device)
        ops.ensure_wgrad_workspace(P["desc"], device)
        self._plans[key] = P
        return P

    def acquire(self, N, H, W, dtype, device):
        P = self._plan(N, H, W, dtype, device)
        if P["free"]:
            return P["free"].pop()
        S = {"P": P}
        S["x"] = torch.empty(N * H * W * self.in_ch, dtype=dtype, device=device)
        S["y"] = torch.empty(N * H * W * self.in_ch, dtype=dtype, device=device)
        S["a"] = [torch.empty(N * (H >> (k + 1)) * (W >> (k + 1)) * self.chans[k], dtype=dtype, device=device)
                  for k in range(4)]
        S["logits"] = torch.empty(N, 1, P["oh"], P["ow"], dtype=torch.float32, device=device)
        S["grads"] = None
        return S

    def release(self, S):
        S["P"]["free"].append(S)

    def _to_nhwc(self, t, dst, dtype):
        t = t.to(torch.float32)
        t = t.contiguous() if t.shape[1] == 1 else t.permute(0, 2, 3, 1).contiguous()
        if dtype == torch.float32:
            return t.reshape(-1)
        ops.cast(t, dst)
        return dst

    def forward(self, x, y, dtype, y2=None, head: bool = True):
        if not (x.is_cuda and y.is_cuda):
            raise ops.PaiError("Discriminator (HIP) needs HIP device tensors; there is no CPU path")
        N, C, H, W = x.shape
        if C != self.in_ch or y.shape != x.shape or (y2 is not None and y2.shape != x.shape):
            raise ops.PaiError(f"Discriminator expects [N,{self.in_ch},H,W] tensors of one shape, got {tuple(x.shape)} "
                               f"and {tuple(y.shape)}")
        reps = 1 if y2 is None else 2
        S = self.acquire(N * reps, H, W, dtype, x.device)
        P = S["P"]
        if y2 is None and dtype != torch.float32 and C == 1:
            ops.cast_multi([(x.detach().to(torch.float32).contiguous().reshape(-1), S["x"]),
                            (y.detach().to(torch.float32).contiguous().reshape(-1), S["y"])])
            S["xin"], S["yin"] = S["x"], S["y"]
        elif y2 is None:
            S["xin"] = self._to_nhwc(x, S["x"], dtype)
            S["yin"] = self._to_nhwc(y, S["y"], dtype)
        else:
            half = N * H * W * C
            pairs = []
            for src, dst in ((x, S["x"][:half]), (x, S["x"][half:]), (y, S["y"][:half]), (y2, S["y"][half:])):
                t = src.detach().to(torch.float32)
                t = t.contiguous() if C == 1 else t.permute(0, 2, 3, 1).contiguous()
                pairs.append((t.reshape(-1), dst))
            ops.cast_multi(pairs)
            S["xin"], S["yin"] = S["x"], S["y"]
        refresh_packs(self.packs, dtype)
        wf, _ = self.packs[0].get(dtype)
        ops.conv_fwd(P["desc"][0], S["xin"], S["yin"], wf, self.convs[0].bias, y_act=S["a"][0])
        for k in range(1, 4):
            wf, _ = self.packs[k].get(dtype)
            ops.conv_fwd(P["desc"][k], S["a"][k - 1], None, wf, self.convs[k].bias, y_act=S["a"][k])
        S["head_done"] = False
        if not head:
            return None, S
        wf, _ = self.packs[4].get(dtype)
        S["logits"] = torch.empty_like(S["logits"])
        ops.conv_fwd(P["desc"][4], S["a"][3], None, wf, None, y_f32=S["logits"])
        return S["logits"], S

    @staticmethod
    def fused_enabled() -> bool:
        return os.environ.get("PAI_HEAD_FUSED", "1") not in ("", "0")

    def head_fused_ok(self, dtype) -> bool:
        return dtype == torch.bfloat16 and self.fused_enabled() and self.convs[4].bias is None

    def _grads(self, S):
        if S["grads"] is None:
            P = S["P"]
            S["grads"] = {"du": [torch.empty_like(a) for a in S["a"]],
                          "dl": torch.empty(S["logits"].numel(), dtype=P["dtype"], device=P["device"]),
                          "dl32": torch.empty(S["logits"].numel(), dtype=torch.float32, device=P["device"]),
                          "dy": torch.empty(P["N"] * P["H"] * P["W"] * self.in_ch, dtype=P["dtype"], device=P["device"])}
        return S["grads"]

    def forward_loss(self, x, y, dtype, y2, n_first, target_first, target_rest, acc, need_grad: bool):
        if not (x.is_cuda and y.is_cuda):
            raise ops.PaiError("Discriminator (HIP) needs HIP device tensors; there is no CPU path")
        N = x.shape[0] * (1 if y2 is None else 2)
        P = self._plan(N, x.shape[2], x.shape[3], dtype, x.device)
        if not ops.head_loss_ok(P["desc"][4], self.convs[4].bias is not None):
            return None
        _, S = self.forward(x, y, dtype, y2=y2, head=False)
        wf, wd = self.packs[4].get(dtype)
        G = self._grads(S) if need_grad else None
        ops.head_loss(P["desc"][4], S["a"][3], wf, wd if need_grad else None, n_first, target_first, target_rest, 1.0, acc, 1.0,
                      S["logits"], G["dl"] if need_grad else None, G["dl32"] if need_grad else None,
                      G["du"][3] if need_grad else None, ACT_LRELU)
        S["head_done"] = need_grad
        return S

    def _wgrad_desc(self, P, k):
        if os.environ.get("PAI_D_WGRAD_SOLO", "1") in ("", "0"):
            return P["desc"][k]
        solo = P.setdefault("desc_solo", {})
        if k not in solo:
            import copy
            d = copy.copy(P["desc"][k])
            d.hints = 1
            solo[k] = d
        return solo[k]

    def backward(self, S, glogits, need_params: bool, need_dy: bool, fresh: bool = False, head_done: bool = False,
                 addend=None):
        conv_wgrad = ops.conv_wgrad_overwrite_w if fresh else ops.conv_wgrad
        P = S["P"]
        N, H, W, dtype, dev = P["N"], P["H"], P["W"], P["dtype"], P["device"]
        G = self._grads(S)
        A = self.arena() if need_params else None
        hook = self.grad_ready_hook
        if head_done:
            if not S.get("head_done"):
                raise ops.PaiError("DiscEngine.backward(head_done=True) without a forward_loss that kept its gradients")
            dl = G["dl"]
        else:
            glogits = glogits.contiguous().float()
            if dtype == torch.float32:
                dl = glogits.reshape(-1)
            else:
                ops.cast(glogits, G["dl"])
                dl = G["dl"]
        d = P["desc"][4]
        side = self._side
        gy = None
        if need_params:
            with torch.cuda.stream(side.fork(d)):
                ops.conv_wgrad(d, S["a"][3], None, dl, A.seg(self.convs[4].weight), None)
                if hook is not None:
                    hook(A, A.end_of(self.convs[4].weight))
            side.mark_scratch()
        _, wd = self.packs[4].get(dtype)
        if not head_done:
            ops.conv_dgrad_act(d, dl, wd, G["du"][3], None, S["a"][3], ACT_LRELU)
        for k in range(3, -1, -1):
            conv = self.convs[k]
            d = P["desc"][k]
            if need_params and k == 0:
                with torch.cuda.stream(side.fork_tail()):
                    (ops.conv_wgrad if min(_cin_cout(conv)) <= 2 else conv_wgrad)(
                        d, S["xin"], S["yin"], G["du"][0], A.seg(conv.weight), A.seg(conv.bias))
            elif need_params:
                with torch.cuda.stream(side.fork(d)):
                    conv_wgrad(self._wgrad_desc(P, k), S["a"][k - 1], None, G["du"][k], A.seg(conv.weight), A.seg(conv.bias))
                    if hook is not None:
                        hook(A, A.end_of(conv.bias))
            if k > 0:
                _, wd = self.packs[k].get(dtype)
                ops.conv_dgrad_act(d, G["du"][k], wd, G["du"][k - 1], None, S["a"][k - 1], ACT_LRELU)
            elif need_dy:
                _, wd = self.packs[0].get(dtype)
                if addend is not None and self.in_ch == 1 and self.fused_enabled() and addend.dtype == torch.float32 \
                        and addend.is_contiguous() and addend.numel() == N * H * W and ops.conv_dgrad_f32add_ok(d):
                    gy = torch.empty(N * H * W, dtype=torch.float32, device=dev)
                    ops.conv_dgrad_f32add(d, G["du"][0], wd, addend, gy)
                else:
                    ops.conv_dgrad(d, G["du"][0], wd, None, G["dy"], only_c2=True)
        side.join()
        if need_params and hook is not None:
            hook(A, A.end_of(self.convs[0].bias))
        if not need_dy:
            return None
        if gy is not None:
            return gy.view(N, 1, H, W)
        gy = torch.empty(N * H * W * self.in_ch, dtype=torch.float32, device=dev)
        ops.cast(G["dy"], gy)
        gy = gy.view(N, 1, H, W) if self.in_ch == 1 else gy.view(N, H, W, self.in_ch).permute(0, 3, 1, 2)
        if addend is not None:
            if gy.is_contiguous() and gy.numel() % 8 == 0:
                ops.add_act(torch.float32, gy, addend, ops.ACT_NONE, gy)
            else:
                gy = gy + addend
        return gy
```

### thesis-pai-reconstruction_amd/functional.py

```python
from __future__ import annotations

import math

import torch

from . import ops


class _SlotRef:

    def __init__(self, engine, slot):
        self.engine, self.slot = engine, slot

    def take(self):
        if self.slot is None:
            raise ops.PaiError("second backward through the same forward: the engine's activation slot has already "
                               "been consumed (retain_graph is not supported)")
        slot, self.slot = self.slot, None
        return slot

    def __del__(self):
        if self.slot is not None:
            try:
                self.engine.release(self.slot)
# ... 14 lines not shown
            ctx.engine, ctx.ref, ctx.params = engine, _SlotRef(engine, slot), params
        else:
            engine.release(slot)
        return pred

    @staticmethod
    def backward(ctx, gpred):
        engine, slot, params = ctx.engine, ctx.ref.take(), ctx.params
        arena = engine.arena()
        if getattr(engine, "overwrites_weight_grads", False):
            fresh = arena.begin_backward(params, overwrite_weights=True)
            engine.backward(slot, gpred, fresh)
        else:
            arena.begin_backward(params)
            engine.backward(slot, gpred)
        arena.attach(params)
        engine.release(slot)
        return (None,) * (5 + len(params))


class DiscFunction(torch.autograd.Function):
    @staticmethod
    def forward(ctx, x, y, engine, dtype, *params):
        logits, slot = engine.forward(x, y, dtype)
        if ctx.needs_input_grad[0]:
            raise ops.PaiError("gradient w.r.t. the conditioning image is not supported")
        if any(ctx.needs_input_grad):
            ctx.engine, ctx.ref, ctx.params = engine, _SlotRef(engine, slot), params
            ctx.need_dy = ctx.needs_input_grad[1]
            ctx.need_params = any(ctx.needs_input_grad[4:])
        else:
            engine.release(slot)
        return logits

    @staticmethod
    def backward(ctx, glogits):
        engine, slot, params = ctx.engine, ctx.ref.take(), ctx.params
        fresh = False
        if ctx.need_params:
            arena = engine.arena()
            fresh = arena.begin_backward(params, overwrite_weights=True)
        gy = engine.backward(slot, glogits, ctx.need_params, ctx.need_dy, fresh)
        if ctx.need_params:
            arena.attach(params)
        engine.release(slot)
        return (None, gy, None, None) + (None,) * len(params)


class DiscPairsFunction(torch.autograd.Function):

    @staticmethod
    def forward(ctx, x, y_real, y_fake, engine, dtype, *params):
        logits, slot = engine.forward(x, y_real, dtype, y2=y_fake)
        if ctx.needs_input_grad[0] or ctx.needs_input_grad[1] or ctx.needs_input_grad[2]:
            raise ops.PaiError("DiscPairsFunction carries no gradient to its image inputs; detach them")
        if any(ctx.needs_input_grad[5:]):
            ctx.engine, ctx.ref, ctx.params = engine, _SlotRef(engine, slot), params
        else:
            engine.release(slot)
        return logits

    @staticmethod
    def backward(ctx, glogits):
        engine, slot, params = ctx.engine, ctx.ref.take(), ctx.params
        arena = engine.arena()
        fresh = arena.begin_backward(params, overwrite_weights=True)
        engine.backward(slot, glogits, True, False, fresh)
        arena.attach(params)
        engine.release(slot)
        return (None,) * (5 + len(params))


class DiscPairsLossFunction(torch.autograd.Function):

    @staticmethod
    def forward(ctx, x, y_real, y_fake, engine, dtype, *params):
        _check_f32_cuda(x, y_real, y_fake)
        if ctx.needs_input_grad[0] or ctx.needs_input_grad[1] or ctx.needs_input_grad[2]:
            raise ops.PaiError("DiscPairsLossFunction carries no gradient to its image inputs; detach them")
        need = any(ctx.needs_input_grad[5:])
        n = x.shape[0]
        ent = _ACC.get(x.device, "gan_d")
        out = torch.empty((), dtype=torch.float32, device=x.device)
        slot = engine.forward_loss(x, y_real, dtype, y_fake, n, 1.0, 0.0, ent[0], need) if engine.head_fused_ok(dtype) else None
        ctx.fused = slot is not None
        grad = None
        if slot is None:
            logits, slot = engine.forward(x, y_real, dtype, y2=y_fake)
            flat = logits.view(-1)
            k = (flat.numel() // logits.shape[0]) * n
            grad = torch.empty_like(flat) if need else None
            ops.bce_logits(flat[:k], 1.0, 1.0, ent[0], 1.0, grad[:k] if need else None)
            ops.bce_logits(flat[k:], 0.0, 1.0, ent[0], 1.0, grad[k:] if need else None)
        ops.scalar_take(ent[0], out)
        _ACC.taken(ent)
        if need:
            ctx.engine, ctx.ref, ctx.params = engine, _SlotRef(engine, slot), params
            if grad is not None:
                ctx.save_for_backward(grad)
        else:
            engine.release(slot)
        return out

    @staticmethod
    def backward(ctx, gout):
        engine, slot, params = ctx.engine, ctx.ref.take(), ctx.params
        arena = engine.arena()
        fresh = arena.begin_backward(params, overwrite_weights=True)
        if ctx.fused and _is_unit(gout):
            engine.backward(slot, None, True, False, fresh, head_done=True)
        else:
            grad = slot["grads"]["dl32"] if ctx.fused else ctx.saved_tensors[0]
            engine.backward(slot, _scaled(grad, gout).view(slot["logits"].shape), True, False, fresh)
        arena.attach(params)
        engine.release(slot)
        return (None,) * (5 + len(params))


class DiscGenLossFunction(torch.autograd.Function):

    @staticmethod
    def forward(ctx, x, pred, target, engine, dtype, l1_weight, *params):
        _check_f32_cuda(x, pred, target)
        if ctx.needs_input_grad[0] or ctx.needs_input_grad[2]:
            raise ops.PaiError("gradient w.r.t. the conditioning image / the target is not supported")
        pc, tc = pred.contiguous().float(), target.contiguous().float()
        need_pred, need_params = ctx.needs_input_grad[1], any(ctx.needs_input_grad[6:])
        need = need_pred or need_params
        gp = torch.empty_like(pc) if need_pred else None
        ent = _ACC.get(pc.device, "gan_g")
        slot = engine.forward_loss(x, pred, dtype, None, x.shape[0], 1.0, 1.0, ent[0], need) if engine.head_fused_ok(dtype) else None
        ctx.fused = slot is not None
        gl = None
        if slot is None:
            logits, slot = engine.forward(x, pred, dtype)
            gl = torch.empty_like(logits) if need else None
            ops.bce_logits(logits, 1.0, 1.0, ent[0], 1.0, gl)
        ops.l1(pc, tc, float(l1_weight), ent[0], float(l1_weight), gp)
        out = torch.empty((), dtype=torch.float32, device=pc.device)
        ops.scalar_take(ent[0], out)
        _ACC.taken(ent)
        if need:
            ctx.engine, ctx.ref, ctx.params = engine, _SlotRef(engine, slot), params
            ctx.need_pred, ctx.need_params = need_pred, need_params
            ctx.save_for_backward(*[g for g in (gl, gp) if g is not None])
        else:
            engine.release(slot)
        return out

    @staticmethod
    def backward(ctx, gout):
        engine, slot, params = ctx.engine, ctx.ref.take(), ctx.params
        saved = list(ctx.saved_tensors)
        unit = _is_unit(gout)
        head_done = ctx.fused and unit
        if head_done:
            gl = None
        elif ctx.fused:
            gl = _scaled(slot["grads"]["dl32"], gout).view(slot["logits"].shape)
        else:
            gl = _scaled(saved.pop(0), gout)
        fresh = False
        if ctx.need_params:
            arena = engine.arena()
            fresh = arena.begin_backward(params, overwrite_weights=True)
        addend = saved[0] if ctx.need_pred and unit and engine.fused_enabled() else None
        gy = engine.backward(slot, gl, ctx.need_params, ctx.need_pred, fresh, head_done=head_done, addend=addend)
        if ctx.need_params:
            arena.attach(params)
        engine.release(slot)
        if ctx.need_pred and addend is None:
            gp = _scaled(saved.pop(0), gout)
            if gy.is_contiguous() and gy.numel() % 8 == 0:
                ops.add_act(torch.float32, gy, gp, ops.ACT_NONE, gy)
            else:
                gy = gy + gp
        return (None, gy, None, None, None, None) + (None,) * len(params)


def _check_f32_cuda(*ts):
    for t in ts:
        if not t.is_cuda:
            raise ops.PaiError("pai losses/metrics need HIP device tensors (no CPU fallback exists)")


class _MeanLoss(torch.autograd.Function):

    @staticmethod
    def forward(ctx, kind, x, target):
        _check_f32_cuda(x)
        xc = x.contiguous().float()
        acc = torch.zeros((), dtype=torch.float64, device=x.device)
        need = ctx.needs_input_grad[1]
        grad = torch.empty_like(xc) if need else None
        if kind == "bce":
            ops.bce_logits(xc, float(target), 1.0, acc, 1.0, grad)
        else:
            tc = target.contiguous().float()
            (ops.l1 if kind == "l1" else ops.mse)(xc, tc, 1.0, acc, 1.0, grad)
        if need:
            ctx.save_for_backward(grad)
        return acc.float()

    @staticmethod
    def backward(ctx, gout):
        (grad,) = ctx.saved_tensors
        return None, _scaled(grad, gout), None


class _Accumulators:

    def __init__(self):
        self.bufs = {}

# ... 370 lines not shown
```

### thesis-pai-reconstruction_amd/lib.py

```python
from __future__ import annotations

import ctypes as C
import os

HERE = os.path.dirname(os.path.abspath(__file__))
LIB_PATH = os.environ.get("PAI_HIP_LIB") or os.path.join(HERE, "libpai_hip.so")

F32, BF16 = 0, 1
U8 = 2
ACT_NONE, ACT_LRELU, ACT_RELU, ACT_TANH = 0, 1, 2, 3
ACT_SILU = 4
HINT_SOLO = 1


class PaiError(RuntimeError):
    pass


class ConvDesc(C.Structure):
    _fields_ = [("dtype", C.c_int32), ("transposed", C.c_int32),
                ("N", C.c_int32), ("H", C.c_int32), ("W", C.c_int32),
                ("C1", C.c_int32), ("C2", C.c_int32), ("Cout", C.c_int32),
                ("kernel", C.c_int32), ("stride", C.c_int32), ("pad", C.c_int32),
                ("relu1", C.c_int32), ("relu2", C.c_int32), ("epilogue_act", C.c_int32),
                ("groups", C.c_int32), ("pack_flags", C.c_int32), ("hints", C.c_int32)]


class BwdEpilogue(C.Structure):
    _fields_ = [("z", C.c_void_p), ("add", C.c_void_p), ("scale", C.c_void_p), ("shift", C.c_void_p),
                ("mean", C.c_void_p), ("rstd", C.c_void_p), ("partials", C.c_void_p),
                ("act1", C.c_int32), ("act2", C.c_int32)]


class BnTrain(C.Structure):
    _fields_ = [("gamma", C.c_void_p), ("beta", C.c_void_p), ("eps", C.c_float), ("momentum", C.c_float),
                ("n_updates", C.c_int32), ("running_mean", C.c_void_p), ("running_var", C.c_void_p),
                ("num_batches_tracked", C.c_void_p), ("mean", C.c_void_p), ("rstd", C.c_void_p),
                ("scale", C.c_void_p), ("shift", C.c_void_p)]


_P = C.c_void_p
_I = C.c_int
_L = C.c_int64
_F = C.c_float
_D = C.POINTER(ConvDesc)

SIGNATURES = {
    "pai_last_error": (C.c_char_p, []),
    "pai_version": (_I, []),
    "pai_device_info": (_I, [C.POINTER(_I), C.POINTER(_I), C.c_char_p, _I]),
    "pai_set_tunable": (_I, [C.c_char_p, _I]),
    "pai_create": (_I, [_I, C.POINTER(C.c_void_p)]),
    "pai_bind": (_I, [C.c_void_p]),
    "pai_destroy": (_I, [C.c_void_p]),
    "pai_handle_set_workspace": (_I, [C.c_void_p, C.c_void_p, C.c_int64]),
    "pai_handle_set_scratch": (_I, [C.c_void_p, C.c_void_p, C.c_int64]),
    "pai_handle_set_wgrad_workspace": (_I, [C.c_void_p, C.c_void_p, C.c_int64]),
    "pai_conv_out_hw": (_I, [_D, C.POINTER(_I), C.POINTER(_I)]),
    "pai_conv_fwd_stats_rows": (_I, [_D]),
    "pai_conv_fwd_stats_rows_max": (_I, [_D]),
    "pai_bn_stats_buffer_rows": (_I, [_I]),
    "pai_conv_kernel_id": (_I, [_D, _I]),
    "pai_conv_kernel_name": (_I, [_D, _I, C.c_char_p, _I]),
    "pai_set_workspace": (_I, [_P, _L]),
    "pai_conv_workspace_bytes": (_L, [_D, _I]),
    "pai_set_scratch": (_I, [_P, _L]),
    "pai_conv_scratch_bytes": (_L, [_D, _I]),
    "pai_set_wgrad_workspace": (_I, [_P, _L]),
    "pai_conv_wgrad_workspace_bytes": (_L, [_D]),
    "pai_conv_fwd": (_I, [_D, _P, _P, _P, _P, _P, _P, _P, _P, _P]),
    "pai_conv_dgrad": (_I, [_D, _P, _P, _P, _P, _I, _P]),
    "pai_conv_dgrad_act": (_I, [_D, _P, _P, _P, _P, _P, _I, _P]),
    "pai_conv_dgrad_f32add_ok": (_I, [_D]),
    "pai_conv_dgrad_f32add": (_I, [_D, _P, _P, _P, _P, _P]),
    "pai_head_loss_ok": (_I, [_D, _I]),
    "pai_head_loss": (_I, [_D, _P, _P, _P, _I, _F, _F, _F, _P, _F, _P, _P, _P, _P, _P, _I, _P]),
    "pai_conv_dgrad_bn_rows_max": (_I, [_D]),
    "pai_conv_dgrad_bn": (_I, [_D, _P, _P, _P, _P, C.POINTER(BwdEpilogue), C.POINTER(_I), _P]),
    "pai_bn_bwd_finalize": (_I, [_P, _I, _I, _P, _P, _P, _P]),
    "pai_conv_fwd_bn": (_I, [_D, _P, _P, _P, _P, _P, _P, _I, C.POINTER(BnTrain), _P, _P]),
    "pai_conv_dgrad_bn_apply": (_I, [_D, _P, _P, _P, _P, C.POINTER(BwdEpilogue), _P, _P, _P, _P, _P, _P]),
    "pai_conv_bn_fused": (_I, [_D, _I]),
    "pai_conv_wgrad": (_I, [_D, _P, _P, _P, _P, _P, _P]),
    "pai_conv_wgrad_overwrite": (_I, [_D, _P, _P, _P, _P, _P, _P]),
    "pai_conv_wgrad_overwrite_w": (_I, [_D, _P, _P, _P, _P, _P, _P]),
    "pai_conv_prologue_ok": (_I, [_D]),
    "pai_conv_fwd_pro": (_I, [_D, _P, _P, _P, _P, _P, _P, _P, _I, _P]),
    "pai_conv_wgrad_pro": (_I, [_D, _P, _P, _P, _P, _I, _P, _P, _I, _P]),
    "pai_pack_weights": (_I, [_I, _P, _I, _I, _I, _P, _P, _P]),
    "pai_build_flags": (_I, []),
    "pai_pack_weights_multi": (_I, [_I, _P, _P, _P, _P, _P, _P, _P]),
    "pai_bn_finalize": (_I, [_P, _I, _I, _L, _P, _P, _F, _F, _I, _P, _P, _P, _P, _P, _P, _P, _P]),
    "pai_bn_eval_coeffs": (_I, [_I, _P, _P, _P, _P, _F, _P, _P, _P]),
    "pai_bn_apply": (_I, [_I, _P, _L, _I, _P, _P, _I, _P, _P]),
    "pai_bn2_add_act": (_I, [_I, _P, _P, _P, _P, _P, _P, _L, _I, _I, _I, _P, _P]),
    "pai_bn_bwd_partial_rows": (_I, [_L]),
    "pai_bn_bwd_reduce": (_I, [_I, _P, _I, _P, _I, _P, _P, _L, _I, _P, _P, _P, _P, _P, _P, _P, _P]),
    "pai_bn_bwd_reduce_affine": (_I, [_I, _P, _I, _P, _I, _P, _L, _I, _P, _P, _P, _P, _P, _P, _P, _P, _P, _P]),
    "pai_bn_bwd_apply": (_I, [_I, _P, _P, _L, _I, _P, _P, _P, _P, _P, _P]),
    "pai_bn_bwd_apply_affine": (_I, [_I, _P, _I, _P, _L, _I, _P, _P, _P, _P, _P, _P, _P, _P]),
    "pai_act_bwd": (_I, [_I, _P, _I, _P, _I, _P, _L, _P, _P]),
    "pai_maxpool2": (_I, [_I, _P, _I, _I, _I, _I, _P, _P, _P]),
    "pai_maxpool2_bwd": (_I, [_I, _P, _P, _I, _I, _I, _I, _P, _P]),
    "pai_upsample2": (_I, [_I, _P, _I, _I, _I, _I, _P, _P]),
    "pai_upsample2_bwd": (_I, [_I, _P, _I, _I, _I, _I, _P, _P]),
    "pai_add_act": (_I, [_I, _P, _P, _L, _I, _P, _P]),
    "pai_bn2_bwd_reduce": (_I, [_I, _P, _I, _P, _P, _L, _I, _P, _P, _P, _P, _P, _P, _P, _P, _P, _P, _P]),
    "pai_bn2_bwd_apply": (_I, [_I, _P, _I, _P, _P, _L, _I, _P, _P, _P, _P, _P, _P, _P, _P, _P, _P, _P, _P, _P]),
    "pai_instnorm_fwd": (_I, [_I, _P, _I, _I, _I, _F, _I, _P, _P, _P, _P]),
    "pai_instnorm_bwd": (_I, [_I, _P, _P, _I, _I, _I, _I, _P, _P, _P, _P]),
    "pai_dropout2d": (_I, [_I, _P, _P, _I, _L, _I, _P, _P]),
    "pai_layernorm_partial_rows": (_I, [_L]),
    "pai_layernorm_fwd": (_I, [_I, _P, _P, _L, _I, _P, _P, _F, _P, _I, _P, _P, _P, _P, _P]),
    "pai_layernorm_bwd": (_I, [_I, _P, _P, _L, _I, _P, _P, _P, _P, _P, _P, _P]),
    "pai_gelu": (_I, [_I, _P, _L, _P, _P]),
    "pai_gelu_bwd": (_I, [_I, _P, _P, _L, _P, _P]),
    "pai_mha_fwd": (_I, [_I, _P, _I, _I, _I, _I, _P, _P, _P, _P]),
    "pai_mha_bwd": (_I, [_I, _P, _P, _P, _I, _I, _I, _I, _P, _P, _P, _P]),
    "pai_mha_kernel_name": (_I, [_I, _I, _I, _I, C.c_char_p, _I]),
    "pai_subsample2": (_I, [_I, _P, _I, _I, _I, _I, _P, _P]),
    "pai_subsample2_bwd": (_I, [_I, _P, _I, _I, _I, _I, _P, _P]),
    "pai_bn_stats_rows": (_I, [_L]),
    "pai_bn_stats": (_I, [_I, _P, _L, _I, _P, _P]),
    "pai_colsum": (_I, [_I, _P, _L, _I, _P, _P]),
    "pai_gate_partial_rows": (_I, [_L]),
    "pai_gate_hidden": (_I, [_I, _P, _P, _L, _I, _P, _P, _P, _P, _P, _P, _P, _P, _P, _P]),
    "pai_gate_apply": (_I, [_I, _P, _P, _L, _I, _P, _P, _P, _P, _P]),
    "pai_gate_apply_bwd": (_I, [_I, _P, _P, _P, _P, _L, _I, _P, _P, _P, _P, _P, _I, _P]),
    "pai_gate_hidden_bwd": (_I, [_I, _P, _P, _P, _P, _P, _L, _I] + [_P] * 15),
    "pai_bce_logits": (_I, [_P, _L, _F, _F, _P, _F, _P, _P]),
    "pai_l1": (_I, [_P, _P, _L, _F, _P, _F, _P, _P]),
    "pai_mse": (_I, [_P, _P, _L, _F, _P, _F, _P, _P]),
    "pai_scalar_take": (_I, [_P, _P, _P]),
    "pai_metrics_take": (_I, [_P, _L, _L, _P, _P]),
    "pai_tanh_bwd": (_I, [_I, _P, _P, _P, _L, _P, _P]),
    "pai_denormalize": (_I, [_P, _P, _L, _P, _P]),
    "pai_ssim_sse": (_I, [_P, _P, _I, _I, _I, _I, _P, _P, _P, _P]),
    "pai_ssim_psnr_bwd": (_I, [_P, _P, _I, _I, _I, _I, _F, _F, _P, _P, _P, _P]),
    "pai_ssim_bwd_workspace_floats": (_L, [_I, _I, _I]),
    "pai_eval_planes": (_I, [_P, _P, _I, _I, _I, _I, _P, _P, _P, _P, _P, _P]),
    "pai_eval_kernel_name": (_I, [_I, C.c_char_p, _I]),
    "pai_cast": (_I, [_I, _P, _I, _P, _L, _P]),
    "pai_reduce_rows": (_I, [_P, _I, _I, _P, _I, _P]),
    "pai_adam": (_I, [_P, _P, _P, _P, _L, _F, _F, _F, _F, _I, _P]),
    "pai_adam_dev": (_I, [_P, _P, _P, _P, _L, _F, _F, _F, _F, _P, _P, _P]),
    "pai_adam_pack": (_I, [_P, _P, _P, _P, _L, _L, _I, _I, _I, _P, _P, _F, _F, _F, _F, _I, _P]),
    "pai_comm_unique_id": (_I, [_P]),
    "pai_comm_init": (_I, [_P, _I, _I, C.POINTER(_P)]),
    "pai_allreduce": (_I, [_P, _P, _L, _I, _P]),
    "pai_comm_destroy": (_I, [_P]),
    "pai_adam_multi": (_I, [_I, _P, _P, _P, _P, _P, _F, _F, _F, _F, _I, _P]),
    "pai_adam_multi_dev": (_I, [_I, _P, _P, _P, _P, _P, _F, _F, _F, _F, _P, _P, _P]),
    "pai_plan_create": (_I, [C.POINTER(_P)]),
    "pai_plan_destroy": (_I, [_P]),
    "pai_plan_begin": (_I, [_P]),
    "pai_plan_end": (_I, [_P]),
    "pai_plan_run": (_I, [_P, _L]),
    "pai_plan_info": (_I, [_P, C.POINTER(_I), C.POINTER(_I), C.POINTER(_I), C.POINTER(_L)]),
    "pai_stream_wait": (_I, [_P, _P]),
# ... 62 lines not shown
```

### thesis-pai-reconstruction_amd/ops.py

```python
from __future__ import annotations

import ctypes as C

import threading
from typing import Optional

import torch

from . import lib as L
from .lib import ACT_LRELU, ACT_NONE, ACT_RELU, ACT_SILU, ACT_TANH, BF16, F32, U8, ConvDesc, PaiError


def code_of(dtype: torch.dtype) -> int:
    if dtype == torch.float32:
        return F32
    if dtype == torch.bfloat16:
        return BF16
    raise PaiError(f"unsupported storage dtype {dtype}")


_TLS = threading.local()


def _stream():
# ... 205 lines not shown
            self._h = C.c_void_p()
            _HANDLES.pop(self.device.index, None) if _HANDLES.get(self.device.index) is self else None


_HANDLES = {}


def handle_for(device) -> Handle:
    dev = torch.device(device)
    idx = dev.index if dev.index is not None else torch.cuda.current_device()
    h = _HANDLES.get(idx)
    if h is None:
        h = _HANDLES[idx] = Handle(torch.device("cuda", idx))
    return h


def conv_workspace_bytes(d: ConvDesc, op: int) -> int:
    return L.load().pai_conv_workspace_bytes(C.byref(d), op)


def ensure_workspace(nbytes: int, device) -> None:
    handle_for(device).ensure_workspace(nbytes)


def conv_scratch_bytes(d: ConvDesc, op: int) -> int:
    return L.load().pai_conv_scratch_bytes(C.byref(d), op)


def scratch_bytes_for(descs) -> int:
    head = max((conv_scratch_bytes(d, op) for d in descs for op in (0, 1)), default=0)
    tail = max((conv_scratch_bytes(d, 2) for d in descs), default=0)
    return head + tail


def ensure_scratch(nbytes: int, device) -> None:
    handle_for(device).ensure_scratch(nbytes)


def conv_wgrad_workspace_bytes(d: ConvDesc) -> int:
    return L.load().pai_conv_wgrad_workspace_bytes(C.byref(d))


def ensure_wgrad_workspace(descs, device) -> None:
    handle_for(device).ensure_wgrad_workspace(max((conv_wgrad_workspace_bytes(d) for d in descs), default=0))


def conv_fwd(d, x1, x2, w, bias, y_raw=None, y_act=None, y_f32=None, stats=None):
    with _Timed(d, 0):
        L.check(L.load().pai_conv_fwd(C.byref(d), _p(x1), _p(x2), _p(w), _p(bias, torch.float32), _p(y_raw),
                                      _p(y_act), _p(y_f32, torch.float32), _p(stats, torch.float32),
                                      _stream()), "pai_conv_fwd")


def conv_prologue_ok(d) -> bool:
    return bool(L.load().pai_conv_prologue_ok(C.byref(d)))


def conv_fwd_pro(d, x1, w, bias, y_raw, stats, pre_scale, pre_shift, pre_act):
    with _Timed(d, 0):
        L.check(L.load().pai_conv_fwd_pro(C.byref(d), _p(x1), _p(w), _p(bias, torch.float32), _p(y_raw),
                                          _p(stats, torch.float32), _p(pre_scale, torch.float32), _p(pre_shift, torch.float32),
                                          int(pre_act), _stream()), "pai_conv_fwd_pro")


def conv_wgrad_pro(d, x1, dy, dw, dbias, overwrite, pre_scale, pre_shift, pre_act):
    with _Timed(d, 2):
        L.check(L.load().pai_conv_wgrad_pro(C.byref(d), _p(x1), _p(dy), _p(dw, torch.float32), _p(dbias, torch.float32),
                                            int(overwrite), _p(pre_scale, torch.float32), _p(pre_shift, torch.float32),
                                            int(pre_act), _stream()), "pai_conv_wgrad_pro")


def conv_dgrad(d, dy, w_dgrad, dx1, dx2=None, only_c2=False):
    with _Timed(d, 1):
        L.check(L.load().pai_conv_dgrad(C.byref(d), _p(dy), _p(w_dgrad), _p(dx1), _p(dx2), int(only_c2),
                                        _stream()), "pai_conv_dgrad")


def conv_dgrad_act(d, dy, w_dgrad, dx1, dx2, a1, act1):
    with _Timed(d, 1):
        L.check(L.load().pai_conv_dgrad_act(C.byref(d), _p(dy), _p(w_dgrad), _p(dx1), _p(dx2), _p(a1), int(act1),
                                            _stream()), "pai_conv_dgrad_act")


def conv_dgrad_f32add_ok(d) -> bool:
    return bool(L.load().pai_conv_dgrad_f32add_ok(C.byref(d)))


def conv_dgrad_f32add(d, dy, w_dgrad, addend, dx2_f32):
    with _Timed(d, 1):
        L.check(L.load().pai_conv_dgrad_f32add(C.byref(d), _p(dy), _p(w_dgrad), _p(addend, torch.float32),
                                               _p(dx2_f32, torch.float32), _stream()), "pai_conv_dgrad_f32add")


def head_loss_ok(d, has_bias: bool = False) -> bool:
    return bool(L.load().pai_head_loss_ok(C.byref(d), int(bool(has_bias))))


def head_loss(d, a3, w_fwd, w_dgrad, n_first, target_first, target_rest, loss_scale, loss, grad_scale, logits, dl=None,
              dl_f32=None, du=None, act=ACT_LRELU):
    L.check(L.load().pai_head_loss(C.byref(d), _p(a3, torch.bfloat16), _p(w_fwd), _p(w_dgrad), int(n_first),
                                   float(target_first), float(target_rest), float(loss_scale), _p(loss, torch.float64),
                                   float(grad_scale), _p(logits, torch.float32), _p(dl, torch.bfloat16),
                                   _p(dl_f32, torch.float32), _p(du, torch.bfloat16), _p(a3) if du is not None else None,
                                   int(act), _stream()), "pai_head_loss")


def conv_dgrad_bn_rows_max(d) -> int:
    return L.load().pai_conv_dgrad_bn_rows_max(C.byref(d))


def conv_dgrad_bn(d, dy, w_dgrad, dx1, dx2, z, act1, add=None, act2=ACT_NONE, scale=None, shift=None,
                  mean=None, rstd=None, partials=None) -> int:
    e = L.BwdEpilogue(_p(z), _p(add), _p(scale, torch.float32), _p(shift, torch.float32), _p(mean, torch.float32),
                      _p(rstd, torch.float32), _p(partials, torch.float32), int(act1), int(act2))
    rows = C.c_int(0)
    with _Timed(d, 1):
        L.check(L.load().pai_conv_dgrad_bn(C.byref(d), _p(dy), _p(w_dgrad), _p(dx1), _p(dx2), C.byref(e),
                                           C.byref(rows), _stream()), "pai_conv_dgrad_bn")
    return rows.value


def conv_fwd_bn(d, x1, x2, w, bias, z, a, act, gamma, beta, eps, momentum, n_updates, running_mean, running_var,
                num_batches_tracked, mean, rstd, scale, shift, stats):
    f32 = torch.float32
    bn = L.BnTrain(_p(gamma, f32), _p(beta, f32), float(eps), float(momentum), int(n_updates), _p(running_mean, f32),
                   _p(running_var, f32), _p(num_batches_tracked, torch.int64), _p(mean, f32), _p(rstd, f32),
                   _p(scale, f32), _p(shift, f32))
    with _Timed(d, 0):
        L.check(L.load().pai_conv_fwd_bn(C.byref(d), _p(x1), _p(x2), _p(w), _p(bias, f32), _p(z), _p(a), int(act),
                                         C.byref(bn), _p(stats, f32), _stream()), "pai_conv_fwd_bn")


def conv_bn_fused(d, op: int) -> bool:
    return L.load().pai_conv_bn_fused(C.byref(d), op) == 1


def conv_dgrad_bn_apply(d, dy, w_dgrad, du_scratch, dx2, z, act1, add, act2, scale, shift, mean, rstd, partials, gamma,
                        sums, dgamma, dbeta, dz):
    f32 = torch.float32
    e = L.BwdEpilogue(_p(z), _p(add), _p(scale, f32), _p(shift, f32), _p(mean, f32), _p(rstd, f32), _p(partials, f32),
                      int(act1), int(act2))
    with _Timed(d, 1):
        L.check(L.load().pai_conv_dgrad_bn_apply(C.byref(d), _p(dy), _p(w_dgrad), _p(du_scratch), _p(dx2), C.byref(e),
                                                 _p(gamma, f32), _p(sums, f32), _p(dgamma, f32), _p(dbeta, f32), _p(dz),
                                                 _stream()), "pai_conv_dgrad_bn_apply")


def bn_bwd_finalize(partials, rows, C_, sums, dgamma, dbeta):
    L.check(L.load().pai_bn_bwd_finalize(_p(partials, torch.float32), rows, C_, _p(sums, torch.float32),
                                         _p(dgamma, torch.float32), _p(dbeta, torch.float32), _stream()),
            "pai_bn_bwd_finalize")


def conv_wgrad(d, x1, x2, dy, dw, dbias=None):
    with _Timed(d, 2):
        L.check(L.load().pai_conv_wgrad(C.byref(d), _p(x1), _p(x2), _p(dy), _p(dw, torch.float32),
                                        _p(dbias, torch.float32), _stream()), "pai_conv_wgrad")


def conv_wgrad_overwrite(d, x1, x2, dy, dw, dbias=None):
    with _Timed(d, 2):
        L.check(L.load().pai_conv_wgrad_overwrite(C.byref(d), _p(x1), _p(x2), _p(dy), _p(dw, torch.float32),
                                                  _p(dbias, torch.float32), _stream()), "pai_conv_wgrad_overwrite")


def conv_wgrad_overwrite_w(d, x1, x2, dy, dw, dbias=None):
    with _Timed(d, 2):
        L.check(L.load().pai_conv_wgrad_overwrite_w(C.byref(d), _p(x1), _p(x2), _p(dy), _p(dw, torch.float32),
                                                    _p(dbias, torch.float32), _stream()), "pai_conv_wgrad_overwrite_w")


def pack_weights(dtype, w_master, Cout, taps, Cin, w_fwd=None, w_dgrad=None):
    L.check(L.load().pai_pack_weights(code_of(dtype), _p(w_master, torch.float32), Cout, taps, Cin, _p(w_fwd),
                                      _p(w_dgrad), _stream()), "pai_pack_weights")


TUNABLE_UNSET = -2147483648


def set_tunable(name: str, value: int = TUNABLE_UNSET) -> None:
    L.check(L.load().pai_set_tunable(name.encode(), int(value)), "pai_set_tunable")


def pack_weights_multi(items):
    import ctypes as C
    n = len(items)
    if n == 0:
# ... 693 lines not shown
```

Before: 11520 images/s.

## Fuse discriminator bias-gradient column sums into dgrad and head-loss epilogues

Adds a column-sum mode to the MFMA dgrad epilogue and to the fused head-loss kernel. Each tile writes per-row-block partial sums of the activation-masked gradient, and a small finalize kernel reduces them into the bias gradient. The wgrad kernels for the discriminator layers no longer need to compute dbias, which removes a separate full read of the gradient tensor. The cost is extra partial-sum buffers, one finalize launch per layer, and more template variants in the epilogue.

```diff
diff --git a/include/pai_hip.h b/include/pai_hip.h
--- a/include/pai_hip.h
+++ b/include/pai_hip.h
@@ -77,6 +77,12 @@
 
 int pai_conv_dgrad_act(const pai_conv_desc* d, const void* dy, const void* w_dgrad, void* dx1,
                        void* dx2, const void* a1, int act1, void* stream);
+
+int pai_conv_dgrad_act_colsum_ok(const pai_conv_desc* d);
+int pai_conv_dgrad_act_colsum(const pai_conv_desc* d, const void* dy, const void* w_dgrad, void* dx1, void* dx2,
+                              const void* a1, int act1, float* partials, int* partial_rows, void* stream);
+int pai_colsum_buffer_rows(int rows);
+int pai_colsum_finalize(const float* partials, int rows, int C, float* out, int accumulate, void* stream);
 
 typedef struct pai_bwd_epilogue {
     const void* z;
@@ -222,10 +228,12 @@
            float grad_scale, float* grad, void* stream);
 int pai_mse(const float* pred, const float* target, int64_t numel, float loss_scale, double* loss,
             float grad_scale, float* grad, void* stream);
+int pai_head_loss_colsum_rows_max(const pai_conv_desc* d);
 int pai_head_loss_ok(const pai_conv_desc* d, int has_bias);
 int pai_head_loss(const pai_conv_desc* d, const void* a3, const void* w_fwd, const void* w_dgrad, int n_first,
                   float target_first, float target_rest, float loss_scale, double* loss, float grad_scale,
-                  float* logits, void* dl, float* dl_f32, void* du, const void* act_src, int act, void* stream);
+                  float* logits, void* dl, float* dl_f32, void* du, const void* act_src, int act, float* du_colsum,
+                  int* du_colsum_rows, void* stream);
 int pai_scalar_take(double* acc, float* out, void* stream);
 int pai_metrics_take(double* sums, int64_t n_images, int64_t numel, float* out3, void* stream);
 int pai_tanh_bwd(int dtype, const float* pred, const float* g_a, const float* g_b, int64_t numel,
diff --git a/thesis-pai-reconstruction_amd/csrc/api.hip b/thesis-pai-reconstruction_amd/csrc/api.hip
--- a/thesis-pai-reconstruction_amd/csrc/api.hip
+++ b/thesis-pai-reconstruction_amd/csrc/api.hip
@@ -12,7 +12,7 @@
 }
 
 extern "C" const char* pai_last_error(void) { return g_err; }
-extern "C" int pai_version(void) { return 140; }
+extern "C" int pai_version(void) { return 141; }
 
 extern "C" int pai_build_flags(void) { return 0; }
 
@@ -646,6 +646,50 @@
     return pai_act_bwd(d->dtype, dx1, act1, nullptr, PAI_ACT_NONE, a1, (int64_t)g.N * g.OH * g.OW * g.D1, dx1, stream);
 }
 
+int launch_colsum(int dtype, const void* x, int64_t rows, int C, float* out, hipStream_t s);
+static bool dgrad_colsum_pick(int dtype, const GG& g, FwdArgs* a, const void* a1, int act1, float* partials, FwdPick* p) {
+    if (!pai_tunable("dbias_fused", 1) || !pick_fwd(dtype, g, *a).fused) return false;
+    FwdArgs f = *a;
+    f.bz = a1; f.bact1 = act1; f.bpart = partials;
+    *p = pick_fwd(dtype, g, f);
+    if (p->k != FK_MFMA) return false;
+    *a = f;
+    return true;
+}
+
+extern "C" int pai_conv_dgrad_act_colsum_ok(const pai_conv_desc* d) {
+    GG g;
+    if (!d || gg_build_dgrad(d, &g)) return 0;
+    FwdArgs a = query_args(g, 1);
+    FwdPick p;
+    return dgrad_colsum_pick(d->dtype, g, &a, (const void*)1, PAI_ACT_LRELU, (float*)1, &p) ? 1 : 0;
+}
+
+extern "C" int pai_conv_dgrad_act_colsum(const pai_conv_desc* d, const void* dy, const void* w_dgrad, void* dx1, void* dx2,
+                                         const void* a1, int act1, float* partials, int* partial_rows, void* stream) {
+    GG g;
+    if (gg_build_dgrad(d, &g)) return 1;
+    PAI_CHECK(dy && w_dgrad && dx1 && a1, "pai_conv_dgrad_act_colsum: null pointer");
+    PAI_CHECK(partials && partial_rows, "pai_conv_dgrad_act_colsum: null partials / partial_rows");
+    PAI_CHECK(d->C2 == 0 || dx2, "pai_conv_dgrad_act_colsum: C2 > 0 but dx2 is null");
+    PAI_CHECK(act1 == PAI_ACT_LRELU || act1 == PAI_ACT_RELU || act1 == PAI_ACT_NONE, "pai_conv_dgrad_act_colsum: act1=%d", act1);
+    FwdArgs a;
+    memset(&a, 0, sizeof(a));
+    a.x1 = dy; a.w = w_dgrad;
+    a.y1 = dx1; a.y2 = dx2;
+    hipStream_t s = (hipStream_t)stream;
+    FwdPick p;
+    if (dgrad_colsum_pick(d->dtype, g, &a, a1, act1, partials, &p)) {
+        *partial_rows = p.rows;
+        return run_fwd(p, d->dtype, g, a, s);
+    }
+    *partial_rows = 1;
+    if (int rc = pai_conv_dgrad_act(d, dy, w_dgrad, dx1, dx2, a1, act1, stream)) return rc;
+    const hipError_t e = pai::memset_async(partials, 0, (size_t)g.D1 * sizeof(float), s);
+    PAI_CHECK(e == hipSuccess, "pai_conv_dgrad_act_colsum: hipMemsetAsync: %s", hipGetErrorString(e));
+    return launch_colsum(d->dtype, dx1, (int64_t)g.N * g.OH * g.OW, g.D1, partials, s);
+}
+
 extern "C" int pai_conv_dgrad_bn_rows_max(const pai_conv_desc* d) {
     GG g;
     if (gg_build_dgrad(d, &g)) return -1;
diff --git a/thesis-pai-reconstruction_amd/csrc/gg_mfma.hip b/thesis-pai-reconstruction_amd/csrc/gg_mfma.hip
--- a/thesis-pai-reconstruction_amd/csrc/gg_mfma.hip
+++ b/thesis-pai-reconstruction_amd/csrc/gg_mfma.hip
@@ -305,7 +305,7 @@
     const bool bwd = a.bz && !a.yact && n0 < g.D1;
     const bf16_t* bzp = (const bf16_t*)a.bz;
     const bf16_t* bap = (const bf16_t*)a.badd;
-    const bool bsum = bwd && a.bpart;
+    const int bsum = bwd_sums_state(a, bwd);
     constexpr int CPR = BN / 8;
     constexpr int ORP = NTHR / CPR;
     const int oc = tid % CPR, orow0 = tid / CPR;
@@ -342,10 +342,12 @@
             }
         }
     }
-    if (bsum)
+    if (bsum == SUMS_BN)
         bwd_write_partials<BN, CPR, NTHR / 64>(sstat, bs1, bs2, tid,
                                                a.bpart + ((size_t)(ph * mtiles + bm) * 2) * g.D1 + n0, g.D1,
                                                a.bmean + n0, a.brstd + n0);
+    else if (bsum == SUMS_COL)
+        bwd_write_colsum<BN, CPR, NTHR / 64>(sstat, bs1, tid, a.bpart + (size_t)(ph * mtiles + bm) * g.D1 + n0);
 }
 
 constexpr int FIN_COLS = 128;
@@ -403,7 +405,7 @@
             const bf16_t* bap = (const bf16_t*)a.badd;
             o = bwd_chunk(o, *(const uint4*)((const bf16_t*)a.bz + off),
                           bap ? *(const uint4*)(bap + off) : make_uint4(0, 0, 0, 0), bap != nullptr,
-                          a.bscale != nullptr, a.bpart != nullptr, a.bact1, a.bact2, BP, bs1, bs2);
+                          a.bscale != nullptr, bwd_sums_state(a, true), a.bact1, a.bact2, BP, bs1, bs2);
         }
         *(uint4*)dst = o;
     }
@@ -430,9 +432,13 @@
             float t1 = 0.f, t2 = 0.f;
 #pragma unroll
             for (int r = 0; r < FIN_ROWS; ++r) { t1 += red[0][r][tid]; t2 += red[1][r][tid]; }
-            float* dst = a.bpart + ((size_t)(ph * mtiles + bm) * 2) * g.D1 + c;
-            dst[0] = t1;
-            dst[g.D1] = a.brstd[c] * (t2 - a.bmean[c] * t1);
+            if (a.bmean) {
+                float* dst = a.bpart + ((size_t)(ph * mtiles + bm) * 2) * g.D1 + c;
+                dst[0] = t1;
+                dst[g.D1] = a.brstd[c] * (t2 - a.bmean[c] * t1);
+            } else {
+                a.bpart[(size_t)(ph * mtiles + bm) * g.D1 + c] = t1;
+            }
         }
     }
 }
@@ -761,7 +767,7 @@
     const bool bwd = a.bz && !a.yact && n0 < g.D1;
     const bf16_t* bzp = (const bf16_t*)a.bz;
     const bf16_t* bap = (const bf16_t*)a.badd;
-    const bool bsum = bwd && a.bpart;
+    const int bsum = bwd_sums_state(a, bwd);
     constexpr int CPR = BN / 8;
     constexpr int ORP = NTHR / CPR;
     static_assert(ORP % 16 == 0, "a pass covers whole 16-pixel tile rows");
@@ -850,7 +856,8 @@
         dst[g.Cout] = q;
     }
     auto store_tile = [&](auto bwd_tag, auto add_tag, auto sum_tag) {
-        constexpr bool BWD = decltype(bwd_tag)::value, ADD = decltype(add_tag)::value, SUM = decltype(sum_tag)::value;
+        constexpr bool BWD = decltype(bwd_tag)::value, ADD = decltype(add_tag)::value;
+        constexpr int SUM = decltype(sum_tag)::value;
         auto request = [&](int pass, int slot) {
             const unsigned off = toff + (unsigned)pass * pstep;
             if (BWD && !(EPI_ABL & 1)) zq[slot] = *(const uint4*)(zt + off);
@@ -873,13 +880,19 @@
     };
     typedef std::true_type T_;
     typedef std::false_type F_;
-    if (!bwd) store_tile(F_{}, F_{}, F_{});
-    else if (bap) { if (bsum) store_tile(T_{}, T_{}, T_{}); else store_tile(T_{}, T_{}, F_{}); }
-    else { if (bsum) store_tile(T_{}, F_{}, T_{}); else store_tile(T_{}, F_{}, F_{}); }
-    if (bsum)
+    typedef std::integral_constant<int, SUMS_NONE> SN_;
+    typedef std::integral_constant<int, SUMS_BN> SB_;
+    typedef std::integral_constant<int, SUMS_COL> SC_;
+    if (!bwd) store_tile(F_{}, F_{}, SN_{});
+    else if (bap) { if (bsum) store_tile(T_{}, T_{}, SB_{}); else store_tile(T_{}, T_{}, SN_{}); }
+    else if (bsum == SUMS_COL) store_tile(T_{}, F_{}, SC_{});
+    else { if (bsum) store_tile(T_{}, F_{}, SB_{}); else store_tile(T_{}, F_{}, SN_{}); }
+    if (bsum == SUMS_BN)
         bwd_write_partials<BN, CPR, NTHR / 64>(sstat, bs1, bs2, tid,
                                                a.bpart + ((size_t)(ph * mtiles + bm) * 2) * g.D1 + n0, g.D1,
                                                a.bmean + n0, a.brstd + n0);
+    else if (bsum == SUMS_COL)
+        bwd_write_colsum<BN, CPR, NTHR / 64>(sstat, bs1, tid, a.bpart + (size_t)(ph * mtiles + bm) * g.D1 + n0);
 }
 
 template <int BM, int BN, bool DBB>
diff --git a/thesis-pai-reconstruction_amd/csrc/gg_tile.h b/thesis-pai-reconstruction_amd/csrc/gg_tile.h
--- a/thesis-pai-reconstruction_amd/csrc/gg_tile.h
+++ b/thesis-pai-reconstruction_amd/csrc/gg_tile.h
@@ -62,7 +62,8 @@
     const float sg = slope == 0.f ? 0.f : fmaf(g, slope, 0.f);
     return pos ? g : sg;
 }
-template <bool HAS_ADD, bool SUMS>
+enum BwdSums { SUMS_NONE = 0, SUMS_BN = 1, SUMS_COL = 2 };
+template <bool HAS_ADD, int SUMS>
 __device__ __forceinline__ uint4 bwd_chunk_t(uint4 gq, uint4 zq, uint4 aq, float sl1, float sl2, const BwdParams& P,
                                              float* s1, float* s2) {
     const unsigned gw[4] = {gq.x, gq.y, gq.z, gq.w}, zw[4] = {zq.x, zq.y, zq.z, zq.w}, aw[4] = {aq.x, aq.y, aq.z, aq.w};
@@ -79,23 +80,29 @@
             d1 += bwd_sel(__uint_as_float(aw[k] & 0xffff0000u), q1, sl2);
         }
         o[k] = pk2bf(d0, d1);
-        if (SUMS) {
+        if (SUMS != SUMS_NONE) {
             const float r0 = __uint_as_float(o[k] << 16), r1 = __uint_as_float(o[k] & 0xffff0000u);
             s1[2 * k] += r0;
             s1[2 * k + 1] += r1;
-            s2[2 * k] = fmaf(r0, z0, s2[2 * k]);
-            s2[2 * k + 1] = fmaf(r1, z1, s2[2 * k + 1]);
+            if (SUMS == SUMS_BN) {
+                s2[2 * k] = fmaf(r0, z0, s2[2 * k]);
+                s2[2 * k + 1] = fmaf(r1, z1, s2[2 * k + 1]);
+            }
         }
     }
     return make_uint4(o[0], o[1], o[2], o[3]);
 }
-__device__ __forceinline__ uint4 bwd_chunk(uint4 gq, uint4 zq, uint4 aq, bool has_add, bool , bool sums,
+__device__ __forceinline__ uint4 bwd_chunk(uint4 gq, uint4 zq, uint4 aq, bool has_add, bool , int sums,
                                            int act1, int act2, const BwdParams& P, float* s1, float* s2) {
     const float sl1 = act_slope(act1), sl2 = act_slope(act2);
-    if (has_add) return sums ? bwd_chunk_t<true, true>(gq, zq, aq, sl1, sl2, P, s1, s2)
-                             : bwd_chunk_t<true, false>(gq, zq, aq, sl1, sl2, P, s1, s2);
-    return sums ? bwd_chunk_t<false, true>(gq, zq, aq, sl1, sl2, P, s1, s2)
-                : bwd_chunk_t<false, false>(gq, zq, aq, sl1, sl2, P, s1, s2);
+    if (has_add) return sums ? bwd_chunk_t<true, SUMS_BN>(gq, zq, aq, sl1, sl2, P, s1, s2)
+                             : bwd_chunk_t<true, SUMS_NONE>(gq, zq, aq, sl1, sl2, P, s1, s2);
+    if (sums == SUMS_COL) return bwd_chunk_t<false, SUMS_COL>(gq, zq, aq, sl1, sl2, P, s1, s2);
+    return sums ? bwd_chunk_t<false, SUMS_BN>(gq, zq, aq, sl1, sl2, P, s1, s2)
+                : bwd_chunk_t<false, SUMS_NONE>(gq, zq, aq, sl1, sl2, P, s1, s2);
+}
+__device__ __forceinline__ int bwd_sums_state(const FwdArgs& a, bool bwd) {
+    return bwd && a.bpart ? (a.bmean ? SUMS_BN : SUMS_COL) : SUMS_NONE;
 }
 template <int BN, int CPR, int NW>
 __device__ __forceinline__ void bwd_write_partials(float* sred, const float* s1, const float* s2, int tid,
@@ -118,6 +125,25 @@
         for (int w = 0; w < NW; ++w) { a += sred[(w * 2 + 0) * BN + tid]; b += sred[(w * 2 + 1) * BN + tid]; }
         row_dst[tid] = a;
         row_dst[D1 + tid] = rstd[tid] * (b - mean[tid] * a);
+    }
+}
+
+template <int BN, int CPR, int NW>
+__device__ __forceinline__ void bwd_write_colsum(float* sred, const float* s1, int tid, float* row_dst) {
+    const int lane = tid & 63, wid = tid >> 6;
+#pragma unroll
+    for (int k = 0; k < 8; ++k) {
+        float a = s1[k];
+#pragma unroll
+        for (int o = CPR; o < 64; o <<= 1) a += __shfl_xor(a, o, 64);
+        if (lane < CPR) sred[wid * BN + lane * 8 + k] = a;
+    }
+    __syncthreads();
+    if (tid < BN) {
+        float a = 0.f;
+#pragma unroll
+        for (int w = 0; w < NW; ++w) a += sred[w * BN + tid];
+        row_dst[tid] = a;
     }
 }
 
diff --git a/thesis-pai-reconstruction_amd/csrc/head.hip b/thesis-pai-reconstruction_amd/csrc/head.hip
--- a/thesis-pai-reconstruction_amd/csrc/head.hip
+++ b/thesis-pai-reconstruction_amd/csrc/head.hip
@@ -16,6 +16,7 @@
     float* dl32;
     bf16_t* du;
     const bf16_t* act_src;
+    float* du_colsum;
     double* loss;
     int N, H, W, C, OH, OW;
     int n_first;
@@ -27,8 +28,12 @@
     int xcd;
 };
 
-static int64_t head_loss_lds_bytes(int H, int W, int C, bool with_du) {
-    const int64_t ys = (((int64_t)H * W * HL_LD * 4) + 15) & ~(int64_t)15;
+static __host__ __device__ int64_t head_loss_ys_bytes(int P, int C, bool with_colsum) {
+    const int64_t ys = (int64_t)P * HL_LD * 4, cs = with_colsum ? (int64_t)HL_WAVES * C * 4 : 0;
+    return ((ys > cs ? ys : cs) + 15) & ~(int64_t)15;
+}
+static int64_t head_loss_lds_bytes(int H, int W, int C, bool with_du, bool with_colsum = false) {
+    const int64_t ys = head_loss_ys_bytes(H * W, C, with_colsum);
     const int64_t dls = (((int64_t)(H - 1) * (W - 1) * 4) + 15) & ~(int64_t)15;
     return ys + dls + (with_du ? (int64_t)16 * C * 2 : 0);
 }
@@ -39,7 +44,7 @@
     __shared__ double wsum[HL_WAVES];
     const int P = p.H * p.W, Q = p.OH * p.OW;
     float* Ys = (float*)hl_sm;
-    float* dls = (float*)(hl_sm + ((((size_t)P * HL_LD * 4) + 15) & ~(size_t)15));
+    float* dls = (float*)(hl_sm + head_loss_ys_bytes(P, p.C, p.du_colsum != nullptr));
     bf16_t* wt = (bf16_t*)((unsigned char*)dls + ((((size_t)Q * 4) + 15) & ~(size_t)15));
     const int tid = threadIdx.x, lane = tid & 63, wid = tid >> 6;
     const int fr = lane & 15, fq = lane >> 4;
@@ -120,6 +125,9 @@
     const int r0 = (p.H * rg) / p.rg, r1 = (p.H * (rg + 1)) / p.rg;
     const int groups = p.C / 8;
     const int items = (r1 - r0) * p.W * groups;
+    float cs[8];
+#pragma unroll
+    for (int j = 0; j < 8; ++j) cs[j] = 0.f;
     for (int item = tid; item < items; item += HL_THREADS) {
         const int pix = item / groups, cg = item - pix * groups;
         const int ry = pix / p.W, ox = pix - ry * p.W, oy = r0 + ry;
@@ -145,6 +153,29 @@
             acc[j] = p.act == PAI_ACT_NONE ? gq : gq * act_grad(zv[j], p.act);
         }
         V8<bf16_t>::st(p.du + o, acc);
+        if (p.du_colsum) {
+#pragma unroll
+            for (int j = 0; j < 8; ++j) cs[j] += bf2f(f2bf(acc[j]));
+        }
+    }
+    if (!p.du_colsum) return;
+    float* csred = Ys;
+#pragma unroll
+    for (int j = 0; j < 8; ++j) {
+        float v = cs[j];
+        for (int o = groups; o < 64; o <<= 1) v += __shfl_xor(v, o, 64);
+        cs[j] = v;
+    }
+    if (lane < groups) {
+#pragma unroll
+        for (int j = 0; j < 8; ++j) csred[wid * p.C + lane * 8 + j] = cs[j];
+    }
+    __syncthreads();
+    for (int c = tid; c < p.C; c += HL_THREADS) {
+        float t = 0.f;
+#pragma unroll
+        for (int w = 0; w < HL_WAVES; ++w) t += csred[w * p.C + c];
+        p.du_colsum[(size_t)blockIdx.x * p.C + c] = t;
     }
 }
 
@@ -157,22 +188,27 @@
     return head_loss_lds_bytes(d->H, d->W, d->C1, true) <= HL_LDS_MAX;
 }
 
+extern "C" int pai_head_loss_colsum_rows_max(const pai_conv_desc* d) { return d && d->N > 0 && d->H > 0 ? d->N * d->H : -1; }
+
 extern "C" int pai_head_loss_ok(const pai_conv_desc* d, int has_bias) {
     return pai_tunable("head_fused", 1) && head_loss_shape_ok(d, has_bias) ? 1 : 0;
 }
 
 extern "C" int pai_head_loss(const pai_conv_desc* d, const void* a3, const void* w_fwd, const void* w_dgrad, int n_first,
                              float target_first, float target_rest, float loss_scale, double* loss, float grad_scale,
-                             float* logits, void* dl, float* dl_f32, void* du, const void* act_src, int act, void* stream) {
+                             float* logits, void* dl, float* dl_f32, void* du, const void* act_src, int act,
+                             float* du_colsum, int* du_colsum_rows, void* stream) {
     PAI_CHECK(head_loss_shape_ok(d, 0), "pai_head_loss: not a bias-free bf16 k4 s1 p1 C -> 1 head within the LDS bound (ask pai_head_loss_ok)");
     PAI_CHECK(a3 && w_fwd && loss && logits, "pai_head_loss: null pointer");
     PAI_CHECK(!du || (w_dgrad && act_src), "pai_head_loss: du needs w_dgrad and act_src");
     PAI_CHECK(act == PAI_ACT_LRELU || act == PAI_ACT_RELU || act == PAI_ACT_NONE, "pai_head_loss: act=%d", act);
+    PAI_CHECK(!du_colsum || (du && du_colsum_rows), "pai_head_loss: du_colsum needs du and du_colsum_rows");
     HeadLoss p;
     memset(&p, 0, sizeof(p));
     p.a3 = (const bf16_t*)a3; p.wf = (const bf16_t*)w_fwd; p.wd = (const bf16_t*)w_dgrad;
     p.logits = logits; p.dl = (bf16_t*)dl; p.dl32 = dl_f32; p.du = (bf16_t*)du; p.act_src = (const bf16_t*)act_src;
     p.loss = loss;
+    p.du_colsum = du_colsum;
     p.N = d->N; p.H = d->H; p.W = d->W; p.C = d->C1; p.OH = d->H - 1; p.OW = d->W - 1;
     p.n_first = n_first < 0 ? 0 : (n_first > d->N ? d->N : n_first);
     p.t_first = target_first; p.t_rest = target_rest;
@@ -184,8 +220,10 @@
     if (rg < 1) rg = 1;
     if (rg > p.H) rg = p.H;
     p.rg = rg;
+    if (du_colsum_rows) *du_colsum_rows = du_colsum ? p.N * rg : 0;
     p.xcd = (p.N % 8) == 0 ? 1 : 0;
-    const size_t lds = (size_t)head_loss_lds_bytes(p.H, p.W, p.C, du != nullptr);
+    const size_t lds = (size_t)head_loss_lds_bytes(p.H, p.W, p.C, du != nullptr, du_colsum != nullptr);
+    PAI_CHECK((int64_t)lds <= HL_LDS_MAX, "pai_head_loss: %zu bytes of LDS with the column sums", lds);
     const dim3 grid((unsigned)(p.N * rg));
     hipStream_t s = (hipStream_t)stream;
 #define HL_CASE(KK)                                                                                                     \
diff --git a/thesis-pai-reconstruction_amd/csrc/misc.hip b/thesis-pai-reconstruction_amd/csrc/misc.hip
--- a/thesis-pai-reconstruction_amd/csrc/misc.hip
+++ b/thesis-pai-reconstruction_amd/csrc/misc.hip
@@ -277,6 +277,76 @@
     return launch_colsum(dtype, x, rows, C, out, (hipStream_t)stream);
 }
 
+constexpr int CS_CHUNKS = 256;
+constexpr int CS_BIG_ROWS = 512;
+extern "C" int pai_colsum_buffer_rows(int rows) { return rows < 0 ? -1 : rows + 2 * CS_CHUNKS; }
+
+__global__ __launch_bounds__(256) void colsum_chunks_k(const float* part, int R, int C, int per, double* out) {
+    __shared__ double red[256];
+    const int tid = threadIdx.x;
+    const int c0 = blockIdx.y * 256, width = min(C - c0, 256);
+    const int lanes = 256 / width;
+    const int cl = tid % width, rl = tid / width;
+    const int r0 = blockIdx.x * per, r1 = min(R, r0 + per);
+    double s0 = 0.0, s1 = 0.0, s2 = 0.0, s3 = 0.0;
+    if (rl < lanes) {
+        const float* src = part + c0 + cl;
+        int r = r0 + rl;
+        for (; r + 3 * lanes < r1; r += 4 * lanes) {
+            const float a = src[(size_t)r * C], b = src[(size_t)(r + lanes) * C];
+            const float c = src[(size_t)(r + 2 * lanes) * C], d = src[(size_t)(r + 3 * lanes) * C];
+            s0 += (double)a; s1 += (double)b; s2 += (double)c; s3 += (double)d;
+        }
+        for (; r < r1; r += lanes) s0 += (double)src[(size_t)r * C];
+    }
+    red[tid] = (s0 + s1) + (s2 + s3);
+    __syncthreads();
+    if (tid < width) {
+        double t = 0.0;
+        for (int l = 0; l < lanes; ++l) t += red[tid + l * width];
+        out[(size_t)blockIdx.x * C + c0 + tid] = t;
+    }
+}
+
+constexpr int CSF_LANES = 128;
+template <typename P>
+__global__ __launch_bounds__(8 * CSF_LANES) void colsum_finalize_k(const P* part, int R, int C, float* out, int accumulate) {
+    __shared__ double red[CSF_LANES / 8][8];
+    const int cl = threadIdx.x & 7, rl = threadIdx.x >> 3;
+    const int c = blockIdx.x * 8 + cl;
+    double s = 0.0;
+    if (c < C)
+        for (int r = rl; r < R; r += CSF_LANES) s += (double)part[(size_t)r * C + c];
+#pragma unroll
+    for (int o = 8; o < 64; o <<= 1) s += __shfl_xor(s, o, 64);
+    if ((threadIdx.x & 63) < 8) red[threadIdx.x >> 6][cl] = s;
+    __syncthreads();
+    if (rl != 0 || c >= C) return;
+    s = 0.0;
+#pragma unroll
+    for (int l = 0; l < CSF_LANES / 8; ++l) s += red[l][cl];
+    out[c] = accumulate ? out[c] + (float)s : (float)s;
+}
+
+extern "C" int pai_colsum_finalize(const float* partials, int rows, int C, float* out, int accumulate, void* stream) {
+    PAI_CHECK(partials && out, "pai_colsum_finalize: null pointer");
+    PAI_CHECK(rows > 0 && C > 0, "pai_colsum_finalize: rows=%d C=%d", rows, C);
+    hipStream_t s = (hipStream_t)stream;
+    if (rows > CS_BIG_ROWS) {
+        PAI_CHECK((C % 2) == 0, "pai_colsum_finalize: %d rows need an even C (fp64 slab sums behind the partials), got %d", rows, C);
+        double* chunks = (double*)(partials + (size_t)rows * C);
+        const int per = cdiv(rows, CS_CHUNKS);
+        PAI_LAUNCH(colsum_chunks_k, dim3(cdiv(rows, per), cdiv(C, 256)), dim3(256), 0, s, partials, rows, C, per, chunks);
+        PAI_LAUNCH_CHECK();
+        PAI_LAUNCH(colsum_finalize_k<double>, dim3(cdiv(C, 8)), dim3(8 * CSF_LANES), 0, s, (const double*)chunks, cdiv(rows, per), C,
+                   out, accumulate);
+    } else {
+        PAI_LAUNCH(colsum_finalize_k<float>, dim3(cdiv(C, 8)), dim3(8 * CSF_LANES), 0, s, partials, rows, C, out, accumulate);
+    }
+    PAI_LAUNCH_CHECK();
+    return 0;
+}
+
 __device__ __forceinline__ void adam1(float& p, float& m, float& v, float g, float lr_over_bc1, float beta1, float beta2,
                                       float omb1, float omb2, float eps, float inv_sqrt_bc2) {
 #pragma clang fp contract(off)
diff --git a/thesis-pai-reconstruction_amd/engine.py b/thesis-pai-reconstruction_amd/engine.py
--- a/thesis-pai-reconstruction_amd/engine.py
+++ b/thesis-pai-reconstruction_amd/engine.py
@@ -844,6 +844,18 @@
     def head_fused_ok(self, dtype) -> bool:
         return dtype == torch.bfloat16 and self.fused_enabled() and self.convs[4].bias is None
 
+    @staticmethod
+    def dbias_fused_enabled() -> bool:
+        return os.environ.get("PAI_D_BIAS_FUSED", "0") not in ("", "0")
+
+    def _colsum_ws(self, S, k):
+        cs = self._grads(S).setdefault("cs", {})
+        if k not in cs:
+            P = S["P"]
+            rows = ops.head_loss_colsum_rows_max(P["desc"][4]) if k == 3 else ops.conv_dgrad_bn_rows_max(P["desc"][k + 1])
+            cs[k] = torch.empty(ops.colsum_buffer_rows(rows) * self.chans[k], dtype=torch.float32, device=P["device"])
+        return cs[k]
+
     def _grads(self, S):
         if S["grads"] is None:
             P = S["P"]
@@ -853,7 +865,8 @@
                           "dy": torch.empty(P["N"] * P["H"] * P["W"] * self.in_ch, dtype=P["dtype"], device=P["device"])}
         return S["grads"]
 
-    def forward_loss(self, x, y, dtype, y2, n_first, target_first, target_rest, acc, need_grad: bool):
+    def forward_loss(self, x, y, dtype, y2, n_first, target_first, target_rest, acc, need_grad: bool,
+                     need_params: bool = False):
         if not (x.is_cuda and y.is_cuda):
             raise ops.PaiError("Discriminator (HIP) needs HIP device tensors; there is no CPU path")
         N = x.shape[0] * (1 if y2 is None else 2)
@@ -863,9 +876,11 @@
         _, S = self.forward(x, y, dtype, y2=y2, head=False)
         wf, wd = self.packs[4].get(dtype)
         G = self._grads(S) if need_grad else None
-        ops.head_loss(P["desc"][4], S["a"][3], wf, wd if need_grad else None, n_first, target_first, target_rest, 1.0, acc, 1.0,
-                      S["logits"], G["dl"] if need_grad else None, G["dl32"] if need_grad else None,
-                      G["du"][3] if need_grad else None, ACT_LRELU)
+        cs = self._colsum_ws(S, 3) if need_grad and need_params and self.dbias_fused_enabled() else None
+        S["du3_rows"] = ops.head_loss(P["desc"][4], S["a"][3], wf, wd if need_grad else None, n_first, target_first,
+                                      target_rest, 1.0, acc, 1.0, S["logits"], G["dl"] if need_grad else None,
+                                      G["dl32"] if need_grad else None, G["du"][3] if need_grad else None, ACT_LRELU,
+                                      du_colsum=cs)
         S["head_done"] = need_grad
         return S
 
@@ -902,6 +917,9 @@
         d = P["desc"][4]
         side = self._side
         gy = None
+        fused_bias = need_params and dtype == torch.bfloat16 and self.dbias_fused_enabled() \
+            and not hasattr(getattr(hook, "__self__", None), "subscribe")
+        cs_rows = {3: S.get("du3_rows", 0) if head_done and fused_bias else 0}
         if need_params:
             with torch.cuda.stream(side.fork(d)):
                 ops.conv_wgrad(d, S["a"][3], None, dl, A.seg(self.convs[4].weight), None)
@@ -914,18 +932,26 @@
         for k in range(3, -1, -1):
             conv = self.convs[k]
             d = P["desc"][k]
+            dbias = A.seg(conv.bias) if need_params else None
+            if cs_rows.get(k, 0):
+                ops.colsum_finalize(self._colsum_ws(S, k), cs_rows[k], self.chans[k], dbias, True)
+                dbias = None
             if need_params and k == 0:
                 with torch.cuda.stream(side.fork_tail()):
                     (ops.conv_wgrad if min(_cin_cout(conv)) <= 2 else conv_wgrad)(
                         d, S["xin"], S["yin"], G["du"][0], A.seg(conv.weight), A.seg(conv.bias))
             elif need_params:
                 with torch.cuda.stream(side.fork(d)):
-                    conv_wgrad(self._wgrad_desc(P, k), S["a"][k - 1], None, G["du"][k], A.seg(conv.weight), A.seg(conv.bias))
+                    conv_wgrad(self._wgrad_desc(P, k), S["a"][k - 1], None, G["du"][k], A.seg(conv.weight), dbias)
                     if hook is not None:
                         hook(A, A.end_of(conv.bias))
             if k > 0:
                 _, wd = self.packs[k].get(dtype)
-                ops.conv_dgrad_act(d, G["du"][k], wd, G["du"][k - 1], None, S["a"][k - 1], ACT_LRELU)
+                if fused_bias and k >= 2 and ops.conv_dgrad_act_colsum_ok(d):
+                    cs_rows[k - 1] = ops.conv_dgrad_act_colsum(d, G["du"][k], wd, G["du"][k - 1], None, S["a"][k - 1],
+                                                               ACT_LRELU, self._colsum_ws(S, k - 1))
+                else:
+                    ops.conv_dgrad_act(d, G["du"][k], wd, G["du"][k - 1], None, S["a"][k - 1], ACT_LRELU)
             elif need_dy:
                 _, wd = self.packs[0].get(dtype)
                 if addend is not None and self.in_ch == 1 and self.fused_enabled() and addend.dtype == torch.float32 \
diff --git a/thesis-pai-reconstruction_amd/functional.py b/thesis-pai-reconstruction_amd/functional.py
--- a/thesis-pai-reconstruction_amd/functional.py
+++ b/thesis-pai-reconstruction_amd/functional.py
@@ -120,7 +120,8 @@
         n = x.shape[0]
         ent = _ACC.get(x.device, "gan_d")
         out = torch.empty((), dtype=torch.float32, device=x.device)
-        slot = engine.forward_loss(x, y_real, dtype, y_fake, n, 1.0, 0.0, ent[0], need) if engine.head_fused_ok(dtype) else None
+        slot = engine.forward_loss(x, y_real, dtype, y_fake, n, 1.0, 0.0, ent[0], need, need_params=need) \
+            if engine.head_fused_ok(dtype) else None
         ctx.fused = slot is not None
         grad = None
         if slot is None:
@@ -167,7 +168,8 @@
         need = need_pred or need_params
         gp = torch.empty_like(pc) if need_pred else None
         ent = _ACC.get(pc.device, "gan_g")
-        slot = engine.forward_loss(x, pred, dtype, None, x.shape[0], 1.0, 1.0, ent[0], need) if engine.head_fused_ok(dtype) else None
+        slot = engine.forward_loss(x, pred, dtype, None, x.shape[0], 1.0, 1.0, ent[0], need, need_params=need_params) \
+            if engine.head_fused_ok(dtype) else None
         ctx.fused = slot is not None
         gl = None
         if slot is None:
diff --git a/thesis-pai-reconstruction_amd/lib.py b/thesis-pai-reconstruction_amd/lib.py
--- a/thesis-pai-reconstruction_amd/lib.py
+++ b/thesis-pai-reconstruction_amd/lib.py
@@ -74,7 +74,12 @@
     "pai_conv_dgrad_f32add_ok": (_I, [_D]),
     "pai_conv_dgrad_f32add": (_I, [_D, _P, _P, _P, _P, _P]),
     "pai_head_loss_ok": (_I, [_D, _I]),
-    "pai_head_loss": (_I, [_D, _P, _P, _P, _I, _F, _F, _F, _P, _F, _P, _P, _P, _P, _P, _I, _P]),
+    "pai_head_loss": (_I, [_D, _P, _P, _P, _I, _F, _F, _F, _P, _F, _P, _P, _P, _P, _P, _I, _P, C.POINTER(_I), _P]),
+    "pai_head_loss_colsum_rows_max": (_I, [_D]),
+    "pai_conv_dgrad_act_colsum_ok": (_I, [_D]),
+    "pai_conv_dgrad_act_colsum": (_I, [_D, _P, _P, _P, _P, _P, _I, _P, C.POINTER(_I), _P]),
+    "pai_colsum_buffer_rows": (_I, [_I]),
+    "pai_colsum_finalize": (_I, [_P, _I, _I, _P, _I, _P]),
     "pai_conv_dgrad_bn_rows_max": (_I, [_D]),
     "pai_conv_dgrad_bn": (_I, [_D, _P, _P, _P, _P, C.POINTER(BwdEpilogue), C.POINTER(_I), _P]),
     "pai_bn_bwd_finalize": (_I, [_P, _I, _I, _P, _P, _P, _P]),
diff --git a/thesis-pai-reconstruction_amd/ops.py b/thesis-pai-reconstruction_amd/ops.py
--- a/thesis-pai-reconstruction_amd/ops.py
+++ b/thesis-pai-reconstruction_amd/ops.py
@@ -311,6 +311,32 @@
                                             _stream()), "pai_conv_dgrad_act")
 
 
+def conv_dgrad_act_colsum_ok(d) -> bool:
+    return bool(L.load().pai_conv_dgrad_act_colsum_ok(C.byref(d)))
+
+
+def conv_dgrad_act_colsum(d, dy, w_dgrad, dx1, dx2, a1, act1, partials) -> int:
+    rows = C.c_int(0)
+    with _Timed(d, 1):
+        L.check(L.load().pai_conv_dgrad_act_colsum(C.byref(d), _p(dy), _p(w_dgrad), _p(dx1), _p(dx2), _p(a1), int(act1),
+                                                   _p(partials, torch.float32), C.byref(rows), _stream()),
+                "pai_conv_dgrad_act_colsum")
+    return rows.value
+
+
+def colsum_buffer_rows(rows: int) -> int:
+    return L.load().pai_colsum_buffer_rows(int(rows))
+
+
+def colsum_finalize(partials, rows, C_, out, accumulate: bool):
+    L.check(L.load().pai_colsum_finalize(_p(partials, torch.float32), int(rows), int(C_), _p(out, torch.float32),
+                                         int(bool(accumulate)), _stream()), "pai_colsum_finalize")
+
+
+def head_loss_colsum_rows_max(d) -> int:
+    return L.load().pai_head_loss_colsum_rows_max(C.byref(d))
+
+
 def conv_dgrad_f32add_ok(d) -> bool:
     return bool(L.load().pai_conv_dgrad_f32add_ok(C.byref(d)))
 
@@ -326,12 +352,14 @@
 
 
 def head_loss(d, a3, w_fwd, w_dgrad, n_first, target_first, target_rest, loss_scale, loss, grad_scale, logits, dl=None,
-              dl_f32=None, du=None, act=ACT_LRELU):
+              dl_f32=None, du=None, act=ACT_LRELU, du_colsum=None) -> int:
+    rows = C.c_int(0)
     L.check(L.load().pai_head_loss(C.byref(d), _p(a3, torch.bfloat16), _p(w_fwd), _p(w_dgrad), int(n_first),
                                    float(target_first), float(target_rest), float(loss_scale), _p(loss, torch.float64),
                                    float(grad_scale), _p(logits, torch.float32), _p(dl, torch.bfloat16),
                                    _p(dl_f32, torch.float32), _p(du, torch.bfloat16), _p(a3) if du is not None else None,
-                                   int(act), _stream()), "pai_head_loss")
+                                   int(act), _p(du_colsum, torch.float32), C.byref(rows), _stream()), "pai_head_loss")
+    return rows.value
 
 
 def conv_dgrad_bn_rows_max(d) -> int:
```

Measured after the change: 11490 images/s. About the same (-0.2%).
